# deltaXdeltaQ/QLDPC_Fault_Tolerance

Hardware: AMD Instinct MI355X
Metric: BP-decoded shots/sec (node) on hgp_34_n1600 + % of HBM/LDS roofline (higher is better)
Workload: dtype f64

## Files before the change

### include/qldpc_hip.h

```cpp
#ifndef QLDPC_HIP_H
#define QLDPC_HIP_H

#include <stdint.h>

#ifdef __cplusplus
extern "C" {
#endif

#define QLDPC_ABI_VERSION 1

#define QLDPC_OK 0
#define QLDPC_EINVAL -1
#define QLDPC_EHIP -2
#define QLDPC_ENOMEM -3
#define QLDPC_ENOTSUP -4

#define QLDPC_PRODUCT_SUM 0
#define QLDPC_MIN_SUM 1

#define QLDPC_LOGICAL_X 0
#define QLDPC_LOGICAL_Z 1
#define QLDPC_LOGICAL_TOTAL 2

#define QLDPC_HIST_BINS 1025
// ... 55 lines not shown
int qldpc_osd_gpu_destroy(qldpc_osd_gpu *osd);
int qldpc_osd_gpu_decode(qldpc_osd_gpu *osd, const uint8_t *d_synd, const double *d_post, const uint8_t *d_conv,
                         const uint8_t *d_bp_corr, uint8_t *d_out0, uint8_t *d_outw, int64_t B, void *stream);
typedef struct qldpc_firstmin qldpc_firstmin;
int qldpc_firstmin_create(const qldpc_graph *g, const double *channel_probs, int32_t max_iter,
                          double ms_scaling_factor, int32_t precision, qldpc_firstmin **out);
int qldpc_firstmin_destroy(qldpc_firstmin *fm);
int qldpc_firstmin_decode(qldpc_firstmin *fm, const uint8_t *d_synd, uint8_t *d_corr, int32_t *d_steps, int64_t B,
                          void *stream);

int qldpc_osd_gpu_geometry(const qldpc_osd_gpu *osd, int32_t *row_words, int32_t *window_words, int32_t *threads,
                           int32_t *workgroups);

int qldpc_mc_create(qldpc_bp *dec_x, const qldpc_graph *logical_x, qldpc_bp *dec_z,
                    const qldpc_graph *logical_z, qldpc_mc **out);
int qldpc_mc_destroy(qldpc_mc *mc);

int qldpc_mc_launch(qldpc_mc *mc, double px, double py, double pz, uint64_t seed, uint64_t shot_begin,
                    int64_t shot_count, int32_t logical_mode, const double *d_uniforms, void *d_counters,
                    uint8_t *d_fail, uint8_t *d_err, uint8_t *d_corr, int32_t *d_iters, int32_t grid_blocks,
                    void *stream);

int qldpc_mc_create_staged(qldpc_bp *dec_x, const qldpc_graph *logical_x, qldpc_bp *dec_z,
                           const qldpc_graph *logical_z, qldpc_mc **out);

int qldpc_mc_launch_weight(qldpc_mc *mc, int32_t weight, double px, double py, double pz, uint64_t seed,
                           uint64_t shot_begin, int64_t shot_count, int32_t logical_mode, void *d_counters,
                           uint8_t *d_fail, uint8_t *d_err, uint8_t *d_corr, int32_t *d_iters, void *stream);

int qldpc_mc_run(qldpc_mc *mc, double px, double py, double pz, uint64_t seed, uint64_t shot_begin,
                 int64_t shot_count, int32_t logical_mode, qldpc_counters *out, void *stream);

int qldpc_phenl_create(qldpc_bp *st_x, qldpc_bp *st_z, qldpc_bp *dec2_x, qldpc_bp *dec2_z,
                       const qldpc_graph *logical_x, const qldpc_graph *logical_z, int32_t num_rep, int64_t max_batch,
                       qldpc_phenl **out);
int qldpc_phenl_destroy(qldpc_phenl *ph);
int qldpc_phenl_trace_len(const qldpc_phenl *ph, int32_t num_rounds, int64_t *out);
int qldpc_phenl_launch(qldpc_phenl *ph, double px, double py, double pz, double q, uint64_t seed,
                       uint64_t shot_begin, int64_t shot_count, int32_t num_rounds, int32_t logical_mode,
                       const double *d_uniforms, void *d_counters, uint8_t *d_fail, uint8_t *d_trace, void *stream);

int qldpc_phenl_set_final_osd(qldpc_phenl *ph, qldpc_osd_gpu *osd_x, qldpc_osd_gpu *osd_z);
int qldpc_phenl_set_round_firstmin(qldpc_phenl *ph, qldpc_firstmin *fm_x, qldpc_firstmin *fm_z);

int qldpc_bp_geometry(const qldpc_bp *bp, int32_t *threads, int32_t *vars_per_thread, int32_t *lds_bytes,
                      int32_t *blocks_per_cu);

int qldpc_bp_engine(const qldpc_bp *bp, int32_t *engine);

int qldpc_bp_kernel_id(const qldpc_bp *bp, int32_t *kernel_id, int32_t *row_chunks);

int qldpc_bp_plan(const qldpc_graph *g, const double *channel_probs, int32_t bp_method, int32_t precision,
                  int32_t vars_per_thread, int32_t min_col_slots, int32_t *out, int32_t out_len);

int qldpc_bp_degree3_slots(const qldpc_bp *bp, int32_t *d3k);

int qldpc_bp_create_hbm(qldpc_graph *g, const double *channel_probs, int32_t max_iter, double ms_scaling_factor,
                        int32_t precision, qldpc_bp **out);

int qldpc_bp_create_relay(qldpc_graph *g, const double *channel_probs, int32_t pre_iter, double pre_gamma,
                          int32_t num_legs, int32_t leg_iter, double gamma_lo, double gamma_hi, int32_t stop_nconv,
                          uint64_t gamma_seed, double ms_scaling_factor, int32_t precision, qldpc_bp **out);
int qldpc_relay_gammas(int32_t n, double pre_gamma, int32_t num_legs, double gamma_lo, double gamma_hi,
                       uint64_t gamma_seed, int32_t precision, double *out);
int qldpc_relay_decode_host(int32_t m, int32_t n, const int32_t *row_ptr, const int32_t *col_idx,
                            const double *channel_probs, int32_t pre_iter, double pre_gamma, int32_t num_legs,
                            int32_t leg_iter, double gamma_lo, double gamma_hi, int32_t stop_nconv,
                            uint64_t gamma_seed, double ms_scaling_factor, int32_t precision, const uint8_t *synd,
                            uint8_t *corr, int32_t *iters, uint8_t *conv, int32_t *nsol, int64_t B, int32_t threads);

int qldpc_bp_create_serial(qldpc_graph *g, const double *channel_probs, int32_t max_iter, double ms_scaling_factor,
                           int32_t precision, int32_t soft, qldpc_bp **out);
int qldpc_serial_layers(int32_t m, int32_t n, const int32_t *row_ptr, const int32_t *col_idx, int32_t *layer_out,
                        int32_t *num_layers);
int qldpc_serial_decode_host(int32_t m, int32_t n, const int32_t *row_ptr, const int32_t *col_idx,
                             const double *channel_probs, int32_t max_iter, double ms_scaling_factor,
                             int32_t precision, const uint8_t *synd, uint8_t *corr, int32_t *iters, uint8_t *conv,
                             double *post, int64_t B, int32_t threads);

int qldpc_mc_set_osd(qldpc_mc *mc, qldpc_osd_gpu *osd_x, qldpc_osd_gpu *osd_z);

int qldpc_bp_lds_model(const qldpc_bp *bp, int64_t *out6);
int qldpc_m2s_place_model(const qldpc_graph *g, int32_t anneal_iters, int64_t *out6);
int qldpc_bp_bank_stats(const qldpc_bp *bp, int32_t *before, int32_t *after);

#define QLDPC_COMM_ID_BYTES 128
typedef struct qldpc_comm qldpc_comm;
int qldpc_comm_unique_id(uint8_t *id_out);
int qldpc_comm_init_rank(int device, int32_t nranks, int32_t rank, const uint8_t *id, qldpc_comm **out);
int qldpc_comm_init_all(int32_t ndev, const int32_t *devices, qldpc_comm **out);
int qldpc_comm_rank(const qldpc_comm *comm, int32_t *rank, int32_t *nranks, int32_t *device);
int qldpc_comm_allreduce_counters(qldpc_comm *comm, void *d_counters, void *stream);
int qldpc_comm_allreduce_counters_group(qldpc_comm **comms, void **d_counters, void **streams, int32_t n);
int qldpc_comm_destroy(qldpc_comm *comm);

int qldpc_shard_range(int64_t total, int32_t nparts, int32_t part, int64_t *begin, int64_t *count);
int qldpc_mc_run_sharded(qldpc_mc **mcs, qldpc_comm **comms, int32_t ndev, double px, double py, double pz,
                         uint64_t seed, uint64_t shot_begin, int64_t shot_count, int32_t logical_mode,
                         qldpc_counters *out);

typedef struct qldpc_circ qldpc_circ;
int qldpc_circ_create(const qldpc_graph *dem, const qldpc_graph *dem_obs, const double *probs, qldpc_bp *dec1,
                      const qldpc_graph *h1_space_cor, const qldpc_graph *L1, qldpc_bp *dec2, const qldpc_graph *L2,
                      int32_t num_rounds, int32_t num_rep, int64_t max_batch, qldpc_circ **out);
int qldpc_circ_create_single_shot(const qldpc_graph *dem, const qldpc_graph *dem_obs, const double *probs,
                                  qldpc_bp *dec1, const qldpc_graph *h_space, const qldpc_graph *L1, qldpc_bp *dec2,
                                  const qldpc_graph *L2, int32_t num_cycles, int64_t max_batch, qldpc_circ **out);
int qldpc_circ_set_round_firstmin(qldpc_circ *circ, qldpc_firstmin *fm);
int qldpc_circ_set_final_osd(qldpc_circ *circ, qldpc_osd_gpu *osd_gpu, const qldpc_osd *osd_host);
int qldpc_circ_set_sampler(qldpc_circ *circ, int32_t sampler);
int qldpc_circ_info(const qldpc_circ *circ, int32_t *detectors, int32_t *observables, int32_t *mechanisms);
int qldpc_circ_launch(qldpc_circ *circ, uint64_t seed, uint64_t shot_begin, int64_t shot_count, void *d_counters,
                      uint8_t *d_fail, uint8_t *d_detobs, void *stream);
int qldpc_circ_sample(qldpc_circ *circ, uint64_t seed, uint64_t shot_begin, int64_t shot_count, uint8_t *d_out,
                      void *stream);
int qldpc_circ_destroy(qldpc_circ *circ);

int qldpc_sample_errors(double px, double py, double pz, uint64_t seed, uint64_t shot_begin, int64_t shot_count,
                        int32_t n, const double *d_uniforms, uint8_t *d_err, void *stream);

int qldpc_sample_errors_weight(int32_t weight, double px, double py, double pz, uint64_t seed, uint64_t shot_begin,
                               int64_t shot_count, int32_t n, uint8_t *d_err, void *stream);
int qldpc_sample_errors_weight_host(int32_t weight, double px, double py, double pz, uint64_t seed,
                                    uint64_t shot_begin, int64_t shot_count, int32_t n, uint8_t *err);

typedef struct qldpc_dist qldpc_dist;
int qldpc_dist_create(int device, int32_t rows, int32_t n, int32_t k, const uint64_t *gen_words,
                      const uint64_t *pair_words, qldpc_dist **out);
int qldpc_dist_run_host(qldpc_dist *h, uint64_t seed, uint64_t trial_begin, int64_t trials, int32_t *trial_min,
                        int32_t *best_weight, uint64_t *best_trial, uint64_t *witness_words);
int qldpc_dist_run(qldpc_dist *h, uint64_t seed, uint64_t trial_begin, int64_t trials, int32_t workgroups,
                   int32_t *trial_min, int32_t *best_weight, uint64_t *best_trial, uint64_t *witness_words,
                   void *stream);
int qldpc_dist_geometry(const qldpc_dist *h, int32_t *threads, int32_t *row_words, int32_t *pair_words,
                        int32_t *lds_bytes);
int qldpc_dist_destroy(qldpc_dist *h);

int qldpc_stream_sync(void *stream);

#ifdef __cplusplus
}
#endif
#endif
```

### qldpc_fault_tolerance_amd/_native.py

```python
from __future__ import annotations

import ctypes
import os

PKG_DIR = os.path.dirname(os.path.abspath(__file__))
LIB_PATH = os.environ.get("QLDPC_LIB") or os.path.join(PKG_DIR, "libqldpc_hip.so")
HIST_BINS = 1025

EXPORTED = [
    "qldpc_abi_version", "qldpc_last_error", "qldpc_device_count", "qldpc_graph_create", "qldpc_graph_destroy",
    "qldpc_graph_info", "qldpc_bp_create", "qldpc_bp_destroy", "qldpc_bp_set_channel_probs",
    "qldpc_bp_decode_batch", "qldpc_mc_create", "qldpc_mc_destroy", "qldpc_mc_launch", "qldpc_mc_run",
    "qldpc_bp_geometry", "qldpc_bp_engine", "qldpc_phenl_create", "qldpc_phenl_destroy",
    "qldpc_phenl_trace_len", "qldpc_phenl_launch", "qldpc_bp_degree3_slots", "qldpc_bp_create_soft",
    "qldpc_bp_decode_batch_soft", "qldpc_osd_create", "qldpc_osd_destroy", "qldpc_osd_rank",
    "qldpc_osd_decode_batch", "qldpc_osd_gpu_create", "qldpc_osd_gpu_destroy", "qldpc_osd_gpu_decode", "qldpc_osd_gpu_geometry",
    "qldpc_firstmin_create", "qldpc_firstmin_destroy", "qldpc_firstmin_decode", "qldpc_phenl_set_round_firstmin", "qldpc_phenl_set_final_osd",
    "qldpc_bp_bank_stats", "qldpc_bp_create_hbm", "qldpc_mc_set_osd", "qldpc_comm_unique_id",
    "qldpc_comm_init_rank", "qldpc_comm_init_all", "qldpc_comm_rank", "qldpc_comm_allreduce_counters",
    "qldpc_comm_allreduce_counters_group", "qldpc_comm_destroy", "qldpc_mc_run_sharded", "qldpc_sample_errors",
    "qldpc_stream_sync", "qldpc_bp_kernel_id", "qldpc_build_flags", "qldpc_circ_create", "qldpc_circ_set_final_osd", "qldpc_circ_set_sampler",
    "qldpc_circ_info", "qldpc_circ_launch", "qldpc_circ_sample", "qldpc_circ_destroy",
    "qldpc_shard_range", "qldpc_bp_lds_model", "qldpc_m2s_place_model", "qldpc_bp_plan",
    "qldpc_circ_create_single_shot", "qldpc_circ_set_round_firstmin",
    "qldpc_dist_create", "qldpc_dist_run_host", "qldpc_dist_run", "qldpc_dist_geometry", "qldpc_dist_destroy",
    "qldpc_mc_create_staged", "qldpc_mc_launch_weight", "qldpc_sample_errors_weight",
    "qldpc_sample_errors_weight_host",
    "qldpc_bp_create_relay", "qldpc_relay_gammas", "qldpc_relay_decode_host",
    "qldpc_bp_create_serial", "qldpc_serial_layers", "qldpc_serial_decode_host",
]
BUILD_EXPERIMENTAL = 1
COMM_ID_BYTES = 128


class NativeUnavailable(RuntimeError):
    pass


EINVAL = -1
ENOTSUP = -4


class QldpcError(RuntimeError):

    def __init__(self, msg: str = "", rc: int = 0):
        super().__init__(msg)
        self.rc = rc


class Counters(ctypes.Structure):

    _fields_ = [
        ("shots", ctypes.c_int64),
        ("failures", ctypes.c_int64),
        ("sector_decodes", ctypes.c_int64 * 2),
        ("sector_iters", ctypes.c_int64 * 2),
        ("sector_nonconv", ctypes.c_int64 * 2),
        ("sector_fail", ctypes.c_int64 * 2),
        ("iter_hist", (ctypes.c_int64 * HIST_BINS) * 2),
    ]


COUNTER_WORDS = ctypes.sizeof(Counters) // 8

_lib = None

_vp = ctypes.c_void_p
_i32 = ctypes.c_int32
_i64 = ctypes.c_int64
_u64 = ctypes.c_uint64
_dbl = ctypes.c_double
_pp = ctypes.POINTER(ctypes.c_void_p)


def _declare(L):
    L.qldpc_abi_version.restype = ctypes.c_int
    L.qldpc_abi_version.argtypes = []
    L.qldpc_last_error.restype = ctypes.c_char_p
    L.qldpc_last_error.argtypes = []
    L.qldpc_device_count.restype = ctypes.c_int
    L.qldpc_device_count.argtypes = [ctypes.POINTER(ctypes.c_int)]
    L.qldpc_graph_create.restype = ctypes.c_int
    L.qldpc_graph_create.argtypes = [ctypes.c_int, _i32, _i32, _vp, _vp, _pp]
    L.qldpc_graph_destroy.restype = ctypes.c_int
    L.qldpc_graph_destroy.argtypes = [_vp]
    L.qldpc_graph_info.restype = ctypes.c_int
    L.qldpc_graph_info.argtypes = [_vp] + [ctypes.POINTER(_i32)] * 5
    L.qldpc_bp_create.restype = ctypes.c_int
    L.qldpc_bp_create.argtypes = [_vp, _vp, _i32, _i32, _dbl, _i32, _i32, _i32, _pp]
    L.qldpc_bp_destroy.restype = ctypes.c_int
    L.qldpc_bp_destroy.argtypes = [_vp]
    L.qldpc_bp_set_channel_probs.restype = ctypes.c_int
    L.qldpc_bp_set_channel_probs.argtypes = [_vp, _vp]
    L.qldpc_bp_decode_batch.restype = ctypes.c_int
    L.qldpc_bp_decode_batch.argtypes = [_vp, _vp, _vp, _vp, _vp, _i64, _vp]
    L.qldpc_bp_create_hbm.restype = ctypes.c_int
    L.qldpc_bp_create_hbm.argtypes = [_vp, _vp, _i32, _dbl, _i32, _pp]
    L.qldpc_bp_create_soft.restype = ctypes.c_int
    L.qldpc_bp_create_soft.argtypes = [_vp, _vp, _i32, _dbl, _i32, _pp]
    L.qldpc_bp_decode_batch_soft.restype = ctypes.c_int
    L.qldpc_bp_decode_batch_soft.argtypes = [_vp, _vp, _vp, _vp, _vp, _vp, _i64, _vp]
    L.qldpc_osd_create.restype = ctypes.c_int
    L.qldpc_osd_create.argtypes = [_i32, _i32, _vp, _vp, _vp, _i32, _i32, _pp]
    L.qldpc_osd_destroy.restype = ctypes.c_int
    L.qldpc_osd_destroy.argtypes = [_vp]
    L.qldpc_osd_rank.restype = ctypes.c_int
# ... 13 lines not shown
    L.qldpc_firstmin_decode.restype = ctypes.c_int
    L.qldpc_firstmin_decode.argtypes = [_vp, _vp, _vp, _vp, _i64, _vp]
    L.qldpc_phenl_set_round_firstmin.restype = ctypes.c_int
    L.qldpc_phenl_set_round_firstmin.argtypes = [_vp, _vp, _vp]
    L.qldpc_osd_gpu_geometry.argtypes = [_vp] + [ctypes.POINTER(_i32)] * 4
    L.qldpc_osd_gpu_decode.argtypes = [_vp, _vp, _vp, _vp, _vp, _vp, _vp, _i64, _vp]
    L.qldpc_phenl_set_final_osd.restype = ctypes.c_int
    L.qldpc_phenl_set_final_osd.argtypes = [_vp, _vp, _vp]
    L.qldpc_mc_create.restype = ctypes.c_int
    L.qldpc_mc_create.argtypes = [_vp, _vp, _vp, _vp, _pp]
    L.qldpc_mc_set_osd.restype = ctypes.c_int
    L.qldpc_mc_set_osd.argtypes = [_vp, _vp, _vp]
    L.qldpc_mc_destroy.restype = ctypes.c_int
    L.qldpc_mc_destroy.argtypes = [_vp]
    L.qldpc_mc_launch.restype = ctypes.c_int
    L.qldpc_mc_launch.argtypes = [_vp, _dbl, _dbl, _dbl, _u64, _u64, _i64, _i32, _vp, _vp, _vp, _vp, _vp, _vp,
                                  _i32, _vp]
    L.qldpc_mc_run.restype = ctypes.c_int
    L.qldpc_mc_run.argtypes = [_vp, _dbl, _dbl, _dbl, _u64, _u64, _i64, _i32, ctypes.POINTER(Counters), _vp]
    L.qldpc_bp_geometry.restype = ctypes.c_int
    L.qldpc_bp_geometry.argtypes = [_vp] + [ctypes.POINTER(_i32)] * 4
    L.qldpc_bp_engine.restype = ctypes.c_int
    L.qldpc_bp_engine.argtypes = [_vp, ctypes.POINTER(_i32)]
    L.qldpc_bp_bank_stats.restype = ctypes.c_int
    L.qldpc_bp_bank_stats.argtypes = [_vp, ctypes.POINTER(_i32), ctypes.POINTER(_i32)]
    L.qldpc_bp_degree3_slots.restype = ctypes.c_int
    L.qldpc_bp_degree3_slots.argtypes = [_vp, ctypes.POINTER(_i32)]
    L.qldpc_phenl_create.restype = ctypes.c_int
    L.qldpc_phenl_create.argtypes = [_vp, _vp, _vp, _vp, _vp, _vp, _i32, _i64, _pp]
    L.qldpc_phenl_destroy.restype = ctypes.c_int
    L.qldpc_phenl_destroy.argtypes = [_vp]
    L.qldpc_phenl_trace_len.restype = ctypes.c_int
    L.qldpc_phenl_trace_len.argtypes = [_vp, _i32, ctypes.POINTER(_i64)]
    L.qldpc_phenl_launch.restype = ctypes.c_int
    L.qldpc_phenl_launch.argtypes = [_vp, _dbl, _dbl, _dbl, _dbl, _u64, _u64, _i64, _i32, _i32, _vp, _vp, _vp, _vp,
                                     _vp]
    L.qldpc_comm_unique_id.restype = ctypes.c_int
    L.qldpc_comm_unique_id.argtypes = [_vp]
    L.qldpc_comm_init_rank.restype = ctypes.c_int
    L.qldpc_comm_init_rank.argtypes = [ctypes.c_int, _i32, _i32, _vp, _pp]
    L.qldpc_comm_init_all.restype = ctypes.c_int
    L.qldpc_comm_init_all.argtypes = [_i32, _vp, _pp]
    L.qldpc_comm_rank.restype = ctypes.c_int
    L.qldpc_comm_rank.argtypes = [_vp] + [ctypes.POINTER(_i32)] * 3
    L.qldpc_comm_allreduce_counters.restype = ctypes.c_int
    L.qldpc_comm_allreduce_counters.argtypes = [_vp, _vp, _vp]
    L.qldpc_comm_allreduce_counters_group.restype = ctypes.c_int
    L.qldpc_comm_allreduce_counters_group.argtypes = [_pp, _pp, _pp, _i32]
    L.qldpc_comm_destroy.restype = ctypes.c_int
    L.qldpc_comm_destroy.argtypes = [_vp]
    L.qldpc_mc_run_sharded.restype = ctypes.c_int
    L.qldpc_mc_run_sharded.argtypes = [_pp, _pp, _i32, _dbl, _dbl, _dbl, _u64, _u64, _i64, _i32,
                                       ctypes.POINTER(Counters)]
    L.qldpc_sample_errors.restype = ctypes.c_int
    L.qldpc_sample_errors.argtypes = [_dbl, _dbl, _dbl, _u64, _u64, _i64, _i32, _vp, _vp, _vp]
    L.qldpc_bp_kernel_id.restype = ctypes.c_int
    L.qldpc_bp_kernel_id.argtypes = [_vp, ctypes.POINTER(_i32), ctypes.POINTER(_i32)]
    L.qldpc_bp_plan.restype = ctypes.c_int
    L.qldpc_bp_plan.argtypes = [_vp, _vp, _i32, _i32, _i32, _i32, ctypes.POINTER(_i32), _i32]
    L.qldpc_stream_sync.restype = ctypes.c_int
    L.qldpc_stream_sync.argtypes = [_vp]
    L.qldpc_build_flags.restype = ctypes.c_int
    L.qldpc_build_flags.argtypes = []
    L.qldpc_circ_create.restype = ctypes.c_int
    L.qldpc_circ_create.argtypes = [_vp, _vp, _vp, _vp, _vp, _vp, _vp, _vp, _i32, _i32, _i64, _pp]
    L.qldpc_circ_create_single_shot.restype = ctypes.c_int
    L.qldpc_circ_create_single_shot.argtypes = [_vp, _vp, _vp, _vp, _vp, _vp, _vp, _vp, _i32, _i64, _pp]
    L.qldpc_circ_set_round_firstmin.restype = ctypes.c_int
    L.qldpc_circ_set_round_firstmin.argtypes = [_vp, _vp]
    L.qldpc_circ_set_final_osd.restype = ctypes.c_int
    L.qldpc_circ_set_final_osd.argtypes = [_vp, _vp, _vp]
    L.qldpc_circ_set_sampler.restype = ctypes.c_int
    L.qldpc_circ_set_sampler.argtypes = [_vp, ctypes.c_int32]
    L.qldpc_circ_info.restype = ctypes.c_int
    L.qldpc_circ_info.argtypes = [_vp] + [ctypes.POINTER(_i32)] * 3
    L.qldpc_circ_launch.restype = ctypes.c_int
    L.qldpc_circ_launch.argtypes = [_vp, _u64, _u64, _i64, _vp, _vp, _vp, _vp]
    L.qldpc_circ_sample.restype = ctypes.c_int
    L.qldpc_circ_sample.argtypes = [_vp, _u64, _u64, _i64, _vp, _vp]
    L.qldpc_bp_lds_model.restype = ctypes.c_int
    L.qldpc_bp_lds_model.argtypes = [_vp, ctypes.POINTER(_i64)]
    L.qldpc_m2s_place_model.restype = ctypes.c_int
    L.qldpc_m2s_place_model.argtypes = [_vp, ctypes.c_int32, ctypes.POINTER(_i64)]
    L.qldpc_shard_range.restype = ctypes.c_int
    L.qldpc_shard_range.argtypes = [_i64, _i32, _i32, ctypes.POINTER(_i64), ctypes.POINTER(_i64)]
    L.qldpc_circ_destroy.restype = ctypes.c_int
    L.qldpc_circ_destroy.argtypes = [_vp]
    L.qldpc_dist_create.restype = ctypes.c_int
    L.qldpc_dist_create.argtypes = [ctypes.c_int, _i32, _i32, _i32, _vp, _vp, _pp]
    L.qldpc_dist_run_host.restype = ctypes.c_int
    L.qldpc_dist_run_host.argtypes = [_vp, _u64, _u64, _i64, _vp, ctypes.POINTER(_i32), ctypes.POINTER(_u64), _vp]
    L.qldpc_dist_run.restype = ctypes.c_int
    L.qldpc_dist_run.argtypes = [_vp, _u64, _u64, _i64, _i32, _vp, ctypes.POINTER(_i32), ctypes.POINTER(_u64), _vp,
                                 _vp]
    L.qldpc_dist_geometry.restype = ctypes.c_int
    L.qldpc_dist_geometry.argtypes = [_vp] + [ctypes.POINTER(_i32)] * 4
    L.qldpc_dist_destroy.restype = ctypes.c_int
    L.qldpc_dist_destroy.argtypes = [_vp]
    L.qldpc_mc_create_staged.restype = ctypes.c_int
    L.qldpc_mc_create_staged.argtypes = [_vp, _vp, _vp, _vp, _pp]
    L.qldpc_mc_launch_weight.restype = ctypes.c_int
    L.qldpc_mc_launch_weight.argtypes = [_vp, _i32, _dbl, _dbl, _dbl, _u64, _u64, _i64, _i32, _vp, _vp, _vp, _vp,
                                         _vp, _vp]
    L.qldpc_sample_errors_weight.restype = ctypes.c_int
    L.qldpc_sample_errors_weight.argtypes = [_i32, _dbl, _dbl, _dbl, _u64, _u64, _i64, _i32, _vp, _vp]
    L.qldpc_sample_errors_weight_host.restype = ctypes.c_int
    L.qldpc_sample_errors_weight_host.argtypes = [_i32, _dbl, _dbl, _dbl, _u64, _u64, _i64, _i32, _vp]
    relay = [_i32, _dbl, _i32, _i32, _dbl, _dbl, _i32, _u64, _dbl, _i32]
    L.qldpc_bp_create_relay.restype = ctypes.c_int
    L.qldpc_bp_create_relay.argtypes = [_vp, _vp] + relay + [_pp]
    L.qldpc_relay_gammas.restype = ctypes.c_int
    L.qldpc_relay_gammas.argtypes = [_i32, _dbl, _i32, _dbl, _dbl, _u64, _i32, _vp]
    L.qldpc_relay_decode_host.restype = ctypes.c_int
    L.qldpc_relay_decode_host.argtypes = [_i32, _i32, _vp, _vp, _vp] + relay + [_vp, _vp, _vp, _vp, _vp, _i64, _i32]
    L.qldpc_bp_create_serial.restype = ctypes.c_int
    L.qldpc_bp_create_serial.argtypes = [_vp, _vp, _i32, _dbl, _i32, _i32, _pp]
    L.qldpc_serial_layers.restype = ctypes.c_int
    L.qldpc_serial_layers.argtypes = [_i32, _i32, _vp, _vp, _vp, _vp]
    L.qldpc_serial_decode_host.restype = ctypes.c_int
    L.qldpc_serial_decode_host.argtypes = [_i32, _i32, _vp, _vp, _vp, _i32, _dbl, _i32, _vp, _vp, _vp, _vp, _vp, _i64,
                                           _i32]


def lib():
    global _lib
    if _lib is None:
        if not os.path.exists(LIB_PATH):
            raise NativeUnavailable(
                f"{LIB_PATH} not found: build the HIP extension first (__graft_entry__.build()); "
                "the engine has no CPU fallback")
        import torch

        L = ctypes.CDLL(LIB_PATH)
        _declare(L)
        if L.qldpc_abi_version() != 1:
            raise NativeUnavailable("libqldpc_hip.so ABI version mismatch")
        _lib = L
    return _lib


def check(rc: int, what: str = "") -> None:
    if rc != 0:
        msg = lib().qldpc_last_error().decode(errors="replace")
        raise QldpcError(f"{what} failed (rc={rc}): {msg}", rc)


def experimental_families() -> bool:
    return bool(lib().qldpc_build_flags() & BUILD_EXPERIMENTAL)


def device_count() -> int:
    c = ctypes.c_int(0)
    rc = lib().qldpc_device_count(ctypes.byref(c))
    return c.value if rc == 0 else 0


def require_gpu() -> None:
    if device_count() <= 0:
        raise NativeUnavailable("no HIP device visible: the MI355X engine needs a GPU (no CPU fallback)")
```

### qldpc_fault_tolerance_amd/csrc/bp_reg.h

```cpp
#pragma once

#ifndef QLDPC_TID_LAUNDER
#define QLDPC_TID_LAUNDER 1
#endif
#ifndef QLDPC_STAMPS
#define QLDPC_STAMPS 0
#endif
#ifndef QLDPC_FLIP_BRANCHFREE
#define QLDPC_FLIP_BRANCHFREE 0
#endif
#ifndef QLDPC_FLIPLATE
#define QLDPC_FLIPLATE 0
#endif
#ifndef QLDPC_M2S_MBCNT
#define QLDPC_M2S_MBCNT 0
#endif
#ifndef QLDPC_C2S_PF
#define QLDPC_C2S_PF 2
#endif
#ifndef QLDPC_F32_C2V4
#define QLDPC_F32_C2V4 1
#endif
#ifndef QLDPC_F64_C2V5
#define QLDPC_F64_C2V5 1
#endif
#ifndef QLDPC_ABS_SH2
#define QLDPC_ABS_SH2 1
#endif
#ifndef QLDPC_C2S_W128
#define QLDPC_C2S_W128 1
#endif
#ifndef QLDPC_M2S_UNIL
#define QLDPC_M2S_UNIL 1
#endif
#ifndef QLDPC_M2S_KEEPVA
#define QLDPC_M2S_KEEPVA 1
#endif
#ifndef QLDPC_M2S_RPTR
#define QLDPC_M2S_RPTR 1
#endif
#ifndef QLDPC_RC_RPTR
#define QLDPC_RC_RPTR 1
#endif
#ifndef QLDPC_M2S_ROWPAIR
#define QLDPC_M2S_ROWPAIR 0
#endif
#ifndef QLDPC_M2S_XMASK
#define QLDPC_M2S_XMASK 1
#endif
#include "bp_slot.h"

namespace qldpc {

constexpr int eng_base(int E) { return E % 10; }
constexpr int eng_sh(int E) { return (E / 10) % 10 ? 2 : 0; }
constexpr bool eng_kv64(int E) { return (E / 100) % 10 != 0; }
constexpr int eng_tail(int E) { return (E / 1000) % 10; }
constexpr bool eng_m2s(int E) { return (E / 10000) % 10 == 1 || (E / 10000) % 10 == 4; }
constexpr bool eng_m2v(int E) { return (E / 10000) % 10 == 4; }
template <int D3K>
__host__ __device__ constexpr int m2v_ecnt(int k) { return 3 * (k < D3K ? k : D3K) + 4 * (k > D3K ? k - D3K : 0); }
constexpr int kM2vRows = 4;
constexpr bool eng_fb(int E) { return (E / 10000) % 10 == 2; }
constexpr bool eng_c2s(int E) { return (E / 10000) % 10 == 3; }
constexpr int eng_d2k(int E) { return (E / 100000) % 10; }
constexpr bool eng_nw(int E) { return eng_m2s(E) && !eng_m2v(E) && eng_tail(E) && eng_sh(E) == 2; }
constexpr int kNwSlots = 2;
template <int ENG, int D3K>
__device__ constexpr bool no_edge(int k, int t) {
  return (eng_m2s(ENG) || eng_c2s(ENG) || eng_fb(ENG)) && ((k < D3K && t >= 3) || (k < eng_d2k(ENG) && t >= 2));
}
constexpr bool eng_m2x(int E) { return eng_m2s(E) || eng_c2s(E); }
template <typename T, int ENG>
constexpr int lb_waves(int LB) {
  return LB <= 256 ? (sizeof(T) == 8 ? (eng_m2s(ENG) && (ENG / 100) % 10 == 2 ? 4
                                        : (eng_base(ENG) == 4 || eng_m2x(ENG)) ? 3 : 2) : 4)
                   : (LB <= 512 && (eng_kv64(ENG) || eng_fb(ENG))) ? 4 : 1;
}
__device__ inline unsigned long long qstamp() {
#if QLDPC_STAMPS
  unsigned long long t;
  __builtin_amdgcn_sched_barrier(0);
  asm volatile("s_memtime %0\n\ts_waitcnt lgkmcnt(0)" : "=s"(t) : : "memory");
  __builtin_amdgcn_sched_barrier(0);
  return t;
#else
  return 0;
#endif
}
template <int ENG>
__device__ inline uint32_t ea_cs(uint32_t ea) { return (ea & 0xFFFFu) << eng_sh(ENG); }
template <int ENG>
__device__ inline uint32_t ea_v(uint32_t ea) { return (ea >> 16) << eng_sh(ENG); }

struct RLayout {
  uint32_t v, t, f, sink, lred, total;
};

__host__ __device__ inline RLayout r_layout(int eng, int vslots, int mmax, int tsize, int tail = 0, int m2s = 0,
                                            int fb = 0) {
  RLayout L;
  L.v = eng == 4 ? 0u : (uint32_t)a16((size_t)(mmax + 1) * (m2s == 2 ? 0 : m2s ? 1 : 2) * tsize);
  L.t = L.v + (uint32_t)a16((size_t)vslots * tsize);
  L.f = L.t + (tail ? (uint32_t)a16((size_t)mmax * tsize) : 0u);
  L.sink = L.f + (uint32_t)a16((size_t)(mmax + 1) * (fb ? 1 : 4));
  L.lred = L.sink + (eng == 4 ? 16u : 0u);
  L.total = L.lred + 48;
  return L;
}
__host__ __device__ inline size_t r_lds_bytes(int img, int chunk) {
  return (size_t)img + 2 * a16((size_t)((chunk + 31) / 32) * 4) + 8 * 12;
}

template <typename T>
struct CSEntry {
  using type = Pair<T>;
};

template <typename T>
__device__ inline T& lds_at(unsigned char* smem, uint32_t off) {
  return *reinterpret_cast<T*>(smem + off);
}
template <typename X>
using LdsPtr = __attribute__((address_space(3))) X*;
__device__ inline uint32_t lds_base(unsigned char* smem) {
  return (uint32_t)(uintptr_t)(LdsPtr<unsigned char>)smem;
}
template <int B>
struct LdsWord;
template <>
struct LdsWord<4> {
  typedef uint32_t type;
};
template <>
struct LdsWord<8> {
  typedef uint32_t type __attribute__((ext_vector_type(2)));
};
template <>
struct LdsWord<16> {
  typedef uint32_t type __attribute__((ext_vector_type(4)));
};
// ... 822 lines not shown
      if (TAIL) r.tcur = lds_ld<T, AP>(smem, r.toff);
      r.fcur = lds_ld<uint32_t, AP>(smem, r.fo);
    }
  };
  auto reduce_row = [&](const RowIn& r, int qq) {
    uint32_t s;
    if (FIRST) {
      s = ((r.fcur >> 1) ^ (r.fcur >> 2)) & 1u;
      sbits |= s << qq;
      lds_st<uint32_t, AP>(smem, r.fo, (r.fcur & 4u) | ((r.fcur >> 2) & 1u));
    } else {
      s = (sbits >> qq) & 1u;
      mism |= (int)((r.fcur ^ s) & 1u);
    }
    double f1 = FT<T>::val(FT<T>::kSent), f2 = f1;
    uint32_t px = s ? 0x80000000u : 0u;
    uint32_t aoff = coff[0];
#pragma unroll
    for (int c = 0; c < NCH; ++c) {
#pragma unroll
      for (int k = 0; k < NV; ++k) {
        const double x = V16<T>::get(r.cur[c], k);
        aoff = __builtin_fabs(x) < f1 ? coff[c] + 8u * (uint32_t)k : aoff;
        double t;
        asm("v_max_f64 %0, %1, |%2|" : "=v"(t) : "v"(f1), "v"(x));
        asm("v_min_f64 %0, %1, %2" : "=v"(f2) : "v"(f2), "v"(t));
        asm("v_min_f64 %0, %1, |%2|" : "=v"(f1) : "v"(f1), "v"(x));
      }
      uint32_t p;
      asm("v_bitop3_b32 %0, %1, %2, %3 bitop3:0x96"
          : "=v"(p)
          : "v"(px), "v"((uint32_t)(FT<T>::bits(r.cur[c].x) >> 32)), "v"((uint32_t)(FT<T>::bits(r.cur[c].y) >> 32)));
      px = p;
    }
    uint32_t amin = r.roff + aoff;
    if (TAIL) {
      const double x = (double)r.tcur;
      amin = __builtin_fabs(x) < f1 ? r.toff : amin;
      double t;
      asm("v_max_f64 %0, %1, |%2|" : "=v"(t) : "v"(f1), "v"(x));
      asm("v_min_f64 %0, %1, %2" : "=v"(f2) : "v"(f2), "v"(t));
      asm("v_min_f64 %0, %1, |%2|" : "=v"(f1) : "v"(f1), "v"(x));
      px ^= (uint32_t)(FT<T>::bits(r.tcur) >> 32);
    }
    const U par = (U)(px & 0x80000000u) << 32;
    lds_st<U, AP>(smem, r.co, FT<T>::bits(f1) | par);
    lds_st<U, AP>(smem, amin, FT<T>::bits(f2) | par);
  };
  const uint32_t drb = (uint32_t)TB * rstride, dtp = (uint32_t)TB * (uint32_t)sizeof(T), dfp = 4u * (uint32_t)TB,
                 dcp = (uint32_t)TB * (uint32_t)sizeof(T);
  if constexpr (QLDPC_M2S_ROWPAIR > 0 && TAIL && NCH == 4) {
    for (int i = tid; i < m; i += 2 * TB, q += 2) {
      if constexpr (AP) asm volatile("" : "+v"(rb));
      RowIn a, b;
      load_row(a, i, rb, tp, fp, cp);
      const bool hb = i + TB < m;
      constexpr int PC = QLDPC_M2S_ROWPAIR < NCH ? QLDPC_M2S_ROWPAIR : NCH;
      if (hb) load_row(b, i + TB, rb + drb, tp + dtp, fp + dfp, cp + dcp, 0, PC);
      reduce_row(a, q);
      if (hb) {
        if constexpr (PC < NCH) load_row(b, i + TB, rb + drb, tp + dtp, fp + dfp, cp + dcp, PC, NCH);
        reduce_row(b, q + 1);
      }
      rb += 2 * drb;
      tp += 2 * dtp;
      fp += 2 * dfp;
      cp += 2 * dcp;
    }
  } else {
    for (int i = tid; i < m; i += TB, ++q) {
      if constexpr (AP) asm volatile("" : "+v"(rb));
      RowIn a;
      load_row(a, i, rb, tp, fp, cp);
      reduce_row(a, q);
      rb += drb;
      tp += dtp;
      fp += dfp;
      cp += dcp;
    }
  }
  return mism;
}

template <typename T, bool FIRST>
__device__ inline int m2v_check(unsigned char* smem, const RLayout& Ly, int m, int tid, int TB, uint32_t& sbits,
                                const M2vRows& RW, uint32_t vbase) {
  using U = typename FT<T>::U;
  static_assert(sizeof(T) == 8, "m2v: fp64 only");
  int mism = 0;
#pragma unroll
  for (int q = 0; q < kM2vRows; ++q) {
    const int i = tid + q * TB;
    if (i >= m) break;
    const uint32_t wd[4] = {RW.w[q].x, RW.w[q].y, RW.w[q].z, RW.w[q].w};
    uint32_t a[7];
#pragma unroll
    for (int e = 0; e < 7; ++e) a[e] = vbase + ((e & 1) ? (wd[e >> 1] >> 16) : (wd[e >> 1] & 0xFFFFu));
    double x[7];
#pragma unroll
    for (int e = 0; e < 7; ++e) x[e] = FT<T>::val(lds_ld<U, true>(nullptr, a[e]));
    const uint32_t fo = Ly.f + 4u * (uint32_t)(i + 1);
    const uint32_t fcur = lds_at<uint32_t>(smem, fo);
    uint32_t s;
    if (FIRST) {
      s = ((fcur >> 1) ^ (fcur >> 2)) & 1u;
      sbits |= s << q;
      lds_at<uint32_t>(smem, fo) = (fcur & 4u) | ((fcur >> 2) & 1u);
    } else {
      s = (sbits >> q) & 1u;
      mism |= (int)((fcur ^ s) & 1u);
    }
    double f1 = FT<T>::val(FT<T>::kSent), f2 = f1;
    uint32_t px = s ? 0x80000000u : 0u;
    uint32_t amin = a[0];
#pragma unroll
    for (int e = 0; e < 7; ++e) {
      amin = __builtin_fabs(x[e]) < f1 ? a[e] : amin;
      double t;
      asm("v_max_f64 %0, %1, |%2|" : "=v"(t) : "v"(f1), "v"(x[e]));
      asm("v_min_f64 %0, %1, %2" : "=v"(f2) : "v"(f2), "v"(t));
      asm("v_min_f64 %0, %1, |%2|" : "=v"(f1) : "v"(f1), "v"(x[e]));
    }
#pragma unroll
    for (int e = 0; e + 1 < 7; e += 2) {
      uint32_t p;
      asm("v_bitop3_b32 %0, %1, %2, %3 bitop3:0x96"
          : "=v"(p)
          : "v"(px), "v"((uint32_t)(FT<T>::bits(x[e]) >> 32)), "v"((uint32_t)(FT<T>::bits(x[e + 1]) >> 32)));
      px = p;
    }
    px ^= (uint32_t)(FT<T>::bits(x[6]) >> 32);
    const U par = (U)(px & 0x80000000u) << 32;
    lds_at<U>(smem, (uint32_t)(i + 1) * (uint32_t)sizeof(T)) = FT<T>::bits(f1) | par;
    lds_st<U, true>(nullptr, amin, FT<T>::bits(f2) | par);
  }
  return mism;
}

template <typename T, bool FIRST, int NCH, int TAIL>
__device__ inline int c2s_check(unsigned char* smem, const RLayout& Ly, int m, int wtid, int TB, uint32_t& sbits,
                                T alpha) {
  using U = typename FT<T>::U;
  using VT = typename V16<T>::type;
  constexpr int NV = V16<T>::N;
  static_assert(sizeof(T) == 8, "c2s: fp64 only");
  int mism = 0;
  int q = 0;
  int tid = wtid;
  asm volatile("" : "+v"(tid));
  const uint32_t rstride = (uint32_t)NCH * 16u;
  for (int i = tid; i < m; i += TB, ++q) {
    const uint32_t roff = Ly.v + 16u + (uint32_t)i * rstride;
    VT cur[NCH];
#pragma unroll
    for (int c = 0; c < NCH; ++c) cur[c] = *reinterpret_cast<const VT*>(smem + roff + 16u * (uint32_t)c);
    const uint32_t toff = Ly.t + (uint32_t)i * (uint32_t)sizeof(T);
    T tcur = (T)0;
    if (TAIL) tcur = lds_at<T>(smem, toff);
    const uint32_t fcur = lds_at<uint32_t>(smem, Ly.f + 4u * (uint32_t)(i + 1));
    uint32_t s;
    if (FIRST) {
      s = ((fcur >> 1) ^ (fcur >> 2)) & 1u;
      sbits |= s << q;
      lds_at<uint32_t>(smem, Ly.f + 4u * (uint32_t)(i + 1)) = (fcur & 4u) | ((fcur >> 2) & 1u);
    } else {
      s = (sbits >> q) & 1u;
// ... 204 lines not shown
    lds_at<Pair<T>>(smem, 0) = z;
  }
}

template <typename T>
constexpr int kRowChunks4 = 8 * (int)sizeof(T) / 16;
template <typename T, bool FIRST>
__device__ inline int c_check_any(unsigned char* smem, const RLayout& Ly, int m, int nch, int tid, int TB,
                                  uint32_t& sbits, T alpha) {
  (void)nch;
  return c_check<T, FIRST, kRowChunks4<T>>(smem, Ly, m, tid, TB, sbits, alpha);
}

template <typename T, int DMAX, int VPL, bool MC, int ENG, int D3K, int NCH = 0>
__device__ void r_pass(const SSector& S, int q, long long c0, int cn, unsigned char* smem, const RLayout& Ly,
                       int vslots, int mmax, uint32_t* failmap, unsigned long long* cnt, const SMcArgs* A,
                       const SDecArgs* D, int tid, int TB) {
  using U = typename FT<T>::U;
  constexpr bool KV = RState<T, DMAX, VPL, ENG>::kKeepV;
  const int m = S.m, n = S.n, nch = S.nch;
  int tidp = tid;
#if QLDPC_TID_LAUNDER
  asm volatile("" : "+v"(tidp));
#endif
  RState<T, DMAX, VPL, ENG> R;
  constexpr bool SP = RState<T, DMAX, VPL, ENG>::kSplit;
  const int wbase = (int)__builtin_amdgcn_readfirstlane((uint32_t)tid) & ~63;
  const uint32_t sbase = lds_base(smem);
  r_load<T, DMAX, VPL, ENG>(S, R, Ly, tidp, TB, sbase);
  r_fill<T, ENG>(S, smem, Ly, vslots, mmax, tidp, TB);
  FMap M;
  M.fbase = eng_base(ENG) == 4 ? Ly.f + 4u : Ly.f;
  M.rstart = Ly.v + 16u;
  M.rsh = 4 + __builtin_ctz((unsigned)nch);
  constexpr bool AB = RState<T, DMAX, VPL, ENG>::kAbs;
  if (AB) M.fbase = Ly.f - (sbase >> (eng_fb(ENG) ? 3 : (sizeof(T) == 4 || eng_m2s(ENG)) ? 1 : 2));
  const uint32_t fdelta = eng_base(ENG) == 4 ? Ly.f : M.fbase;
  const bool last_live = eng_nw(ENG) ? ((S.live_last >> ((uint32_t)wbase >> 6)) & 1u) != 0
                                     : uni((VPL - 1) * TB + (tid & ~63) < S.npos ? 1 : 0) != 0;
  uint32_t nwm = 0;
  if constexpr (eng_nw(ENG)) {
    const uint32_t wv = (uint32_t)wbase >> 6;
#pragma unroll
    for (int k = 0; k < kNwSlots && k < VPL; ++k) nwm |= ((S.nw >> (16 * k + wv)) & 1u) << k;
    nwm = __builtin_amdgcn_readfirstlane(nwm);
  }
  uint32_t* lred = reinterpret_cast<uint32_t*>(smem + Ly.lred);
  uint32_t* flags = lred + 8;
  const bool adaptive = S.alpha == 0.0;
  const T alpha_fixed = (T)S.alpha;
  __syncthreads();

  int pshot = -1, pit = 0, pconv = 0;
  unsigned long long st_acc[10] = {0, 0, 0, 0, 0, 0, 0, 0, 0, 0};
  unsigned long long st_a = qstamp();
  for (int sh = 0; sh <= cn; ++sh) {
    const bool have = sh < cn;
    uint32_t eb = 0, sb = 0;
    r_launder<T, DMAX, VPL, ENG, D3K>(R);
    int tidl = tid;
    asm volatile("" : "+v"(tidl));
    if (have) {
#pragma unroll
      for (int k = 0; k < VPL; ++k) {
        const U cl = FT<T>::bits(r_prior(R, k));
#pragma unroll
        for (int t = 0; t < DMAX; ++t) {
          if (no_edge<ENG, D3K>(k, t)) continue;
          if constexpr (eng_m2v(ENG)) {
            if (k == VPL - 1 && tidl >= S.vnl) continue;
            lds_st<U, true>(smem, m2v_va<T, DMAX, VPL, ENG, D3K, 256>(R, k, t), cl);
          }
          else
            lds_st<U, AB>(smem, r_va(R, k, t), cl);
          if (KV) R.ov[KV ? k : 0][KV ? t : 0] = cl;
        }
      }
      if (MC) {
        const long long sl = c0 + sh;
        const unsigned long long gshot = A->shot_begin + (unsigned long long)sl;
        int jv[VPL];
#pragma unroll
        for (int k = 0; k < VPL; ++k) jv[k] = S.perm[k * TB + tidl];
        uint16_t* cc = nullptr;
        bool cc_read = false;
        uint32_t cw = 0;
        if (A->cls_cache && !A->uniforms && VPL <= 8) {
          cc = A->cls_cache + ((long long)blockIdx.x * A->chunk + sh) * TB + tidl;
          cc_read = q == A->sec_id1;
          if (cc_read) cw = *cc;
        }
#pragma unroll
        for (int k = 0; k < VPL; ++k) {
          const int j = jv[k];
          if (j >= 0) {
            uint32_t cls;
            if (A->uniforms) {
              const double u = A->uniforms[sl * (long long)n + j];
              cls = (u < A->t1) ? 2u : (A->t1 <= u && u < A->t2) ? 1u : (A->t2 <= u && u < A->t3) ? 3u : 0u;
            } else if (cc_read) {
              cls = (cw >> (2 * k)) & 3u;
            } else {
              const unsigned long long kk = philox_k53(A->seed, gshot, (uint32_t)j);
              cls = (kk < A->K1) ? 2u : (kk < A->K2) ? 1u : (kk < A->K3) ? 3u : 0u;
              cw |= cls << (2 * k);
            }
            const uint32_t e = (q == 0) ? (cls & 1u) : (cls >> 1);
            eb |= e << k;
            if (A->err && q == A->sec_id0) A->err[sl * (long long)n + j] = (uint8_t)cls;
            if (e) {
#pragma unroll
              for (int t = 0; t < DMAX; ++t) {
                if (no_edge<ENG, D3K>(k, t)) continue;
                if constexpr (eng_base(ENG) == 4)
                  atomicXor(&lds_at<uint32_t>(smem, f_addr<T, ENG>(R.ea[k][t], M)), 2u);
                else if constexpr (eng_c2s(ENG))
                  lds_xor_abs(R.ea[k][t], 2u);
                else
                  f_xor<ENG>(smem, r_fa(R, k, t, M.fbase), 2u);
              }
            }
          }
        }
        if (cc && !cc_read) *cc = (uint16_t)cw;
      } else {
        const uint8_t* srow = D->synd + (c0 + sh) * (long long)m;
        for (int i = tidl; i < m; i += TB) {
          const uint32_t fo = f_off<ENG>(Ly, i + 1);
          const uint32_t F = f_ld<ENG>(smem, fo);
          const int oi = S.rperm ? S.rperm[i] : i;
          f_st<ENG>(smem, fo, (eng_base(ENG) == 4 ? (F & 0xFFFF0000u) : (F & 4u)) | ((uint32_t)(srow[oi] & 1u) << 1));
        }
      }
    }
    if (QLDPC_STAMPS) {
      const unsigned long long t = qstamp();
      st_acc[4] += t - st_a;
      st_a = t;
    }
    M2vRows rwv;
    if constexpr (eng_m2v(ENG))
      if (have) m2v_rows_load(S, tid, TB, m, rwv);
    __syncthreads();
    if (pshot >= 0) {
      uint32_t lf = 0;
      if (MC) {
#pragma unroll
        for (int w = 0; w < 8; ++w) lf |= lred[w];
      }
      const int f = (!pconv || lf) ? 1 : 0;
      if (tid == 0) {
        const long long sl = c0 + pshot;
        if (MC) {
          if (f) failmap[pshot >> 5] |= 1u << (pshot & 31);
          cnt[kCntDec + q] += 1;
          cnt[kCntIters + q] += (unsigned long long)pit;
          cnt[kCntNonconv + q] += pconv ? 0 : 1;
          cnt[kCntSecFail + q] += (unsigned long long)f;
          atomicAdd(&A->counters[kCntHist + q * kHistBins + (pit < kHistBins ? pit : kHistBins - 1)], 1ull);
          if (A->iters) A->iters[sl * 2 + q] = pit;
        } else {
          if (D->iters) D->iters[sl] = pit;
          if (D->conv) D->conv[sl] = pconv ? 1 : 0;
        }
      }
    }
    if (!have) break;
    if (QLDPC_STAMPS) {
      const unsigned long long t = qstamp();
      st_acc[8] += t - st_a;
      st_a = t;
    }
    if constexpr (eng_base(ENG) == 4)
      c_check_any<T, true>(smem, Ly, m, nch, tid, TB, sb, adaptive ? (T)0.5 : alpha_fixed);
    else if constexpr (eng_c2s(ENG))
      c2s_check<T, true, NCH, eng_tail(ENG)>(smem, Ly, m, tid, TB, sb, adaptive ? (T)0.5 : alpha_fixed);
    else if constexpr (eng_m2v(ENG))
      m2v_check<T, true>(smem, Ly, m, tid, TB, sb, rwv, sbase + Ly.v);
    else if constexpr (eng_m2s(ENG))
      m_check<T, true, NCH, eng_tail(ENG)>(smem, Ly, m, wbase, tid, TB, sb);
    else if constexpr (NCH > 0)
      r_check_c<T, true, NCH, eng_tail(ENG), QLDPC_PFC, ENG>(smem, Ly, m, tid, TB, sb);
    else
      r_check<T, true>(smem, Ly, m, nch, tid, TB, sb, adaptive ? (T)0.5 : alpha_fixed);
    __syncthreads();
    if (tid < 10) lred[tid] = 0;
    if (QLDPC_STAMPS) {
      const unsigned long long t = qstamp();
      st_acc[9] += t - st_a;
      st_acc[7] += 1;
      st_a = t;
    }
    int it = 1;
    bool conv = false;
    uint32_t xb = 0;
    uint64_t xm[VPL];
#pragma unroll
    for (int k = 0; k < VPL; ++k) xm[k] = 0;
    long long cslot = -1;
    while (true) {
      int mism;
      double* cpost = nullptr;
      if constexpr (MC && eng_base(ENG) == 3) {
        if (A->c_n && A->c_post[q] && it >= S.max_iter) {
          uint32_t* s_cslot = lred + 11;
          if (tid == 0) *s_cslot = atomicAdd(&A->c_n[q], 1u);
          __syncthreads();
          cslot = (long long)*s_cslot;
          if (cslot < A->c_cap) cpost = A->c_post[q] + cslot * (long long)n;
        }
      }
      if constexpr (eng_base(ENG) == 4) {
        xb = c_var<T, DMAX, VPL>(smem, R, M, last_live);
        __syncthreads();
        const T alpha = adaptive ? (T)(1.0 - ldexp(1.0, -(it + 1))) : alpha_fixed;
        mism = c_check_any<T, false>(smem, Ly, m, nch, tid, TB, sb, alpha);
      } else {
        const T alpha = adaptive ? (T)(1.0 - ldexp(1.0, -it)) : alpha_fixed;
        constexpr int kPV = (eng_tail(ENG) && !eng_m2x(ENG) && !eng_fb(ENG)) ? 0 : QLDPC_PRIO_V;
        if (kPV) __builtin_amdgcn_s_setprio(kPV);
        if constexpr (eng_m2x(ENG))
          xb = m_var<T, DMAX, VPL, D3K, ENG>(smem, R, fdelta, alpha, xb, xm, last_live, cpost, S.perm + tidl, TB, nwm);
        else
          xb = r_var<T, DMAX, VPL, D3K, ENG>(smem, R, fdelta, alpha, xb, last_live, cpost, S.perm + tidl, TB);
        if (kPV) __builtin_amdgcn_s_setprio(0);
        if constexpr (eng_m2v(ENG)) m2v_rows_load(S, tid, TB, m, rwv);
        unsigned long long t1 = 0;
        if (QLDPC_STAMPS) {
          t1 = qstamp();
          st_acc[0] += t1 - st_a;
        }
        __syncthreads();
        if (QLDPC_STAMPS) {
          st_a = qstamp();
          st_acc[1] += st_a - t1;
        }
        const T alpha_next = adaptive ? (T)(1.0 - ldexp(1.0, -(it + 1))) : alpha_fixed;
        if (QLDPC_PRIO_C) __builtin_amdgcn_s_setprio(QLDPC_PRIO_C);
        if constexpr (eng_c2s(ENG))
          mism = c2s_check<T, false, NCH, eng_tail(ENG)>(smem, Ly, m, tid, TB, sb, alpha_next);
        else if constexpr (eng_m2v(ENG))
          mism = m2v_check<T, false>(smem, Ly, m, tid, TB, sb, rwv, sbase + Ly.v);
        else if constexpr (eng_m2s(ENG))
          mism = m_check<T, false, NCH, eng_tail(ENG)>(smem, Ly, m, wbase, tid, TB, sb);
        else if constexpr (NCH > 0)
          mism = r_check_c<T, false, NCH, eng_tail(ENG), QLDPC_PFC, ENG>(smem, Ly, m, tid, TB, sb);
        else
          mism = r_check<T, false>(smem, Ly, m, nch, tid, TB, sb, alpha_next);
        if (QLDPC_PRIO_C) __builtin_amdgcn_s_setprio(0);
        if (QLDPC_STAMPS) {
          const unsigned long long t = qstamp();
          st_acc[2] += t - st_a;
          st_a = t;
        }
      }
      if (__any(mism) && (tid & 63) == 0) flags[it & 1] = 1u;
      __syncthreads();
      if (QLDPC_STAMPS) {
        const unsigned long long t = qstamp();
        st_acc[3] += t - st_a;
        st_acc[6] += 1;
        st_a = t;
      }
      const int any = uni((int)flags[it & 1]);
      if (tid == 0) flags[(it & 1) ^ 1] = 0;
      conv = any == 0;
      if (conv || it >= S.max_iter) break;
      ++it;
    }
    if constexpr (eng_m2x(ENG) && eng_base(ENG) != 4 && m_xmask(ENG)) {
      xb = 0;
#pragma unroll
      for (int k = 0; k < VPL; ++k) xb |= (__builtin_amdgcn_inverse_ballot_w64(xm[k]) ? 1u : 0u) << k;
    }
    const long long sl = c0 + sh;
    if (MC && cslot >= 0 && cslot < A->c_cap) {
      if (!conv) {
        uint8_t* cs = A->c_synd[q] + cslot * (long long)m;
        int qq = 0;
        for (int i = tidl; i < m; i += TB, ++qq)
          cs[S.rperm ? S.rperm[i] : i] =
              (uint8_t)(((sb >> qq) ^ (f_ld<ENG>(smem, f_off<ENG>(Ly, i + 1)) >> 2)) & 1u);
        uint8_t* ce = A->c_err[q] + cslot * (long long)n;
#pragma unroll
        for (int k = 0; k < VPL; ++k) {
          const int j = S.perm[k * TB + tidl];
          if (j >= 0) ce[j] = (uint8_t)((eb >> k) & 1u);
        }
      }
      if (tid == 0) A->c_shot[q][cslot] = conv ? -1 : sl;
    }
    if (MC) {
      const uint32_t r = eb ^ xb;
      if (__any(r != 0)) {
        int jv[VPL];
#pragma unroll
        for (int k = 0; k < VPL; ++k) jv[k] = ((r >> k) & 1u) ? S.perm[k * TB + tidl] : -1;
        const int kw = S.kw;
#pragma unroll
        for (int w = 0; w < 4; ++w) {
          if (w >= kw) break;
          unsigned long long lm[VPL];
#pragma unroll
          for (int k = 0; k < VPL; ++k) lm[k] = jv[k] >= 0 ? S.lmask[(long long)jv[k] * kw + w] : 0ull;
          unsigned long long a = 0;
#pragma unroll
          for (int k = 0; k < VPL; ++k) a ^= lm[k];
          const uint32_t lo = wave_xor_u32((uint32_t)a), hi = wave_xor_u32((uint32_t)(a >> 32));
          if ((tid & 63) == 0) {
            if (lo) atomicXor(&lred[2 * w], lo);
            if (hi) atomicXor(&lred[2 * w + 1], hi);
          }
        }
      }
      if (A->corr) {
#pragma unroll
        for (int k = 0; k < VPL; ++k) {
          const int j = S.perm[k * TB + tidl];
          if (j >= 0) A->corr[(sl * 2 + q) * (long long)n + j] = (uint8_t)((xb >> k) & 1u);
        }
      }
    } else {
#pragma unroll
      for (int k = 0; k < VPL; ++k) {
        const int j = S.perm[k * TB + tidl];
// ... 106 lines not shown
```

### qldpc_fault_tolerance_amd/csrc/bp_slot.h

```cpp
#pragma once
#include "bp_kernels.h"

namespace qldpc {

constexpr int kMaxThreadsS = 1024;
constexpr int kMaxVplS = 32;
constexpr uint32_t kNoEdgeS = 0u;
__device__ inline uint32_t echk(uint32_t e) { return e & 0xFFFFu; }
__device__ inline uint32_t eslot(uint32_t e) { return e >> 16; }

struct SSector {
  const uint32_t* edges;
  const void* llr;
  const unsigned long long* lmask;
  const uint8_t* rdeg;
  const int32_t* perm;
  const int32_t* rperm;
  int m, n, kw, max_iter, nch, vpl;
  int d3k;
  double alpha;
  const uint32_t* rows;
  int vlast, vnl;
  int npos;
  uint32_t nw;
  uint32_t live_last;
};

struct SMcArgs {
  SSector sec[2];
  int nsec, sec_id0, sec_id1, logical_mode;
  int mmax, vslots, img_bytes, chunk;
  unsigned long long K1, K2, K3;
  double t1, t2, t3;
  unsigned long long seed, shot_begin;
  long long shot_count;
  const double* uniforms;
  unsigned long long* counters;
  uint8_t* fail;
  uint8_t* err;
  uint8_t* corr;
  int* iters;
  unsigned int* work;
  unsigned int* c_n;
  double* c_post[2];
  uint8_t* c_synd[2];
  uint8_t* c_err[2];
  long long* c_shot[2];
  long long c_cap;
  unsigned long long* stamps;
  uint16_t* cls_cache;
};

struct SDecArgs {
  SSector sec;
  const uint8_t* synd;
  uint8_t* corr;
  int* iters;
  uint8_t* conv;
  long long B;
  int mmax, vslots, img_bytes, chunk;
  unsigned int* work;
  unsigned long long* stamps;
};

template <typename T> struct V16;
template <> struct V16<float> {
  using type = float4;
  static constexpr int N = 4;
  __device__ static inline float get(const float4& v, int k) { return k == 0 ? v.x : k == 1 ? v.y : k == 2 ? v.z : v.w; }
  __device__ static inline float4 splat(float s) { return make_float4(s, s, s, s); }
};
template <> struct V16<double> {
  using type = double2;
  static constexpr int N = 2;
  __device__ static inline double get(const double2& v, int k) { return k == 0 ? v.x : v.y; }
  __device__ static inline double2 splat(double s) { return make_double2(s, s); }
};

__host__ __device__ inline size_t a16(size_t x) { return (x + 15) & ~(size_t)15; }

__host__ __device__ inline size_t slot_img_bytes(int vslots, int mmax, int tsize) {
  return a16((size_t)vslots * tsize) + a16((size_t)(mmax + 1) * 2 * tsize) + a16((size_t)(mmax + 1) * 4) + 48;
}
__host__ __device__ inline size_t slot_lds_bytes(int ns, int img, int chunk) {
  return (size_t)ns * img + 2 * a16((size_t)((chunk + 31) / 32) * 4) + 8 * 12;
}

template <typename T>
struct Img {
  T* V;
  Pair<T>* CS;
  uint32_t* F;
  uint32_t* lred;
  uint32_t* flags;
};

template <typename T>
__device__ inline Img<T> slot_img(unsigned char* smem, int q, int img_bytes, int vslots, int mmax) {
  unsigned char* b = smem + (size_t)q * img_bytes;
  Img<T> I;
  I.V = reinterpret_cast<T*>(b);
  size_t off = a16((size_t)vslots * sizeof(T));
  I.CS = reinterpret_cast<Pair<T>*>(b + off);
  off += a16((size_t)(mmax + 1) * 2 * sizeof(T));
  I.F = reinterpret_cast<uint32_t*>(b + off);
  off += a16((size_t)(mmax + 1) * 4);
  I.lred = reinterpret_cast<uint32_t*>(b + off);
  I.flags = I.lred + 8;
  return I;
}

template <typename T>
__device__ inline typename FT<T>::U canon(T v) {
  using U = typename FT<T>::U;
  return (FT<T>::bits(v) & ~FT<T>::kSign) | ((v <= (T)0) ? FT<T>::kSign : (U)0);
}

template <int DMAX>
__device__ inline void load_edges(const SSector& S, int k, int tid, int TB, uint32_t (&e)[DMAX]) {
#pragma unroll
  for (int t = 0; t < DMAX; ++t) e[t] = S.edges[(k * DMAX + t) * TB + tid];
}

template <typename T, int DMAX>
__device__ inline void s_priors(const SSector& S, T* V, int tid, int TB) {
  const T* llr = static_cast<const T*>(S.llr);
  for (int k = 0; k < S.vpl; ++k) {
    uint32_t e[DMAX];
    load_edges<DMAX>(S, k, tid, TB, e);
    const T c = FT<T>::val(canon<T>(llr[k * TB + tid]));
#pragma unroll
    for (int t = 0; t < DMAX; ++t) V[eslot(e[t])] = c;
  }
// ... 372 lines not shown
```

### qldpc_fault_tolerance_amd/csrc/qldpc_hip.hip

```cpp
#include <hip/hip_runtime.h>

#include <algorithm>
#include <cmath>
#include <cstdio>
#include <cstdlib>
#include <cstring>
#include <map>
#include <mutex>
#include <string>
#include <vector>

#include "../../include/qldpc_hip.h"
#include "variants.h"
#include "runtime.h"

using namespace qldpc;
using namespace qldpc_rt;

thread_local std::string qldpc_rt::g_err;

namespace {

const int kVplSet[] = {1, 2, 3, 4, 5, 6, 7, 8, 10, 12};
constexpr int kLdsMax = 160 * 1024;
constexpr int kChunkMax = 1024;

int env_int(const char* name, int dflt) {
  const char* e = std::getenv(name);
  return (e && *e) ? std::atoi(e) : dflt;
}

}

namespace {

Variant get_variant(int precision, int vpl, int dmax) {
  if (precision == 32) return dmax == 4 ? get_variant_f32_d4(vpl) : get_variant_f32_d8(vpl);
  return dmax == 4 ? get_variant_f64_d4(vpl) : get_variant_f64_d8(vpl);
}

SVariant get_svariant(int precision, int dmax, int ns) {
  if (precision == 32) return dmax == 4 ? get_svariant_f32_d4(ns) : get_svariant_f32_d8(ns);
  return dmax == 4 ? get_svariant_f64_d4(ns) : get_svariant_f64_d8(ns);
}

SVariant get_rvariant(int engine, int precision, int vpl, int d3k, int dmax) {
  if (engine == 4) return precision == 32 ? get_r4variant_f32(vpl) : get_r4variant_f64(vpl);
  if (precision == 32 && dmax == 5) return get_rvariant_f32_d5(vpl, d3k);
  if (precision == 32 && dmax == 6) return get_rvariant_f32_d6(vpl, d3k);
  return precision == 32 ? get_rvariant_f32(vpl, d3k) : get_rvariant_f64(vpl);
}

bool use_f64w(const Route& r) {
  return r.engine == 3 && r.precision == 64 &&
         (r.DMAX == 4 || (r.DMAX == 5 && (r.VPL <= 5 || (r.VPL == 6 && r.nch == 5)))) && r.ea_shift == 0 && r.TB <= 256 &&
         r.VPL >= 4 && r.VPL <= 8 && (r.nch == 3 || r.nch == 4 || (r.DMAX == 5 && r.nch == 5)) &&
         env_int("QLDPC_F64W", 1) != 0;
}

bool use_f32w(const Route& r) {
  return r.engine == 3 && r.precision == 32 && r.DMAX == 4 && r.ea_shift == 0 && r.VPL >= 5 && r.VPL <= 8 && r.nch == 2 &&
         env_int("QLDPC_F32W", 1) != 0;
}

#if QLDPC_STAMPS
unsigned long long* debug_stamps_buffer() {
  static unsigned long long* buf = nullptr;
  if (!buf && hipMalloc(&buf, 10 * sizeof(unsigned long long)) == hipSuccess) (void)hipMemset(buf, 0, 80);
  return buf;
}
#endif

bool use_f64x(const Route& r) {
  return r.engine == 3 && r.precision == 64 && r.DMAX == 4 && r.ea_shift == 0 && r.TB > 256 && r.TB <= 512 && r.VPL >= 3 &&
         r.VPL <= 4 && QLDPC_EXPERIMENTAL && env_int("QLDPC_F64X", 0) != 0;
}

SVariant slot_variant(const Route& r) {
  const SVariant none{nullptr, nullptr, nullptr, nullptr};
  const bool e3 = r.engine == 3, f64 = r.precision == 64;
  if (r.fb) {
    const bool ok = e3 && !f64 && r.DMAX == 4 && r.ea_shift == 2 && r.nch == 2 && r.tail && r.TB == 512;
    return ok ? get_rvariant_f32_stfb(r.VPL, r.d3k, r.d2k) : none;
  }
  if (r.m2s) {
    if (r.m2s == 1 && e3 && f64 && r.DMAX == 4 && r.ea_shift == 2 && r.nch == 4 && r.tail && r.TB >= 512)
      return get_rvariant_f64_m2st(r.VPL, r.d3k, r.d2k);
    if (r.m2s == 1 && e3 && f64 && r.DMAX == 5 && r.ea_shift == 0 && r.nch == 4 && !r.tail && r.TB <= 256)
      return r.m2s_pk ? get_rvariant_f64_m2s8pk(r.VPL, r.d3k) : get_rvariant_f64_m2s8(r.VPL, r.d3k);
    const bool ok = e3 && f64 && r.DMAX == 4 && r.ea_shift == 0 && r.nch == 3 && r.tail && r.TB <= 256;
    if (r.m2s == 3)
      return (e3 && f64 && r.DMAX == 4 && r.ea_shift == 0 && r.TB == 256) ? get_rvariant_f64_m2v(r.VPL, r.d3k) : none;
    if (!ok) return none;
    return r.m2s == 2 ? get_rvariant_f64_c2s(r.VPL, r.d3k) : get_rvariant_f64_m2s(r.VPL, r.d3k);
  }
  if (r.tail) {
    const bool ok = e3 && r.DMAX == 4 && r.ea_shift == 2 && r.nch == (f64 ? 4 : 2) && (r.TB > 512 || (f64 && r.TB == 512));
    if (!ok) return none;
    return f64 ? get_rvariant_f64_st(r.VPL, r.d3k, r.d2k) : get_rvariant_f32_st(r.VPL, r.d3k);
  }
  if (use_f64w(r)) return r.DMAX == 5 ? get_rvariant_f64_w_d5(r.VPL, r.d3k, r.nch) : get_rvariant_f64_w(r.VPL, r.d3k, r.nch);
  if (use_f64x(r)) return get_rvariant_f64_x(r.VPL, r.d3k);
  if (use_f32w(r)) return get_rvariant_f32_w(r.VPL, r.d3k);
  if (r.engine == 4 && f64 && r.TB <= 256 && r.VPL >= 4) return get_r4variant_f64_w(r.VPL);
  if (e3 && r.ea_shift == 2) return (!f64 && r.DMAX == 4) ? get_rvariant_f32_big(r.VPL, r.d3k) : none;
  return r.engine >= 3 ? get_rvariant(r.engine, r.precision, r.VPL, r.d3k, r.DMAX) : get_svariant(r.precision, r.DMAX, r.NS);
}

int route_kernel_id(const Route& r) {
  if (r.engine != 3) return r.engine;
  if (r.m2s)
    return r.m2s == 2 ? 31103 : r.m2s == 3 ? 40103 : (r.tail && r.nch == 4) ? 11313 + 100000 * std::min(r.d2k, 1)
           : r.tail ? 11103 : r.m2s_pk ? 10203 : 10103;
  if (r.fb) return 21013 + ((r.d3k >= 8 && r.d2k > 0) ? 100000 * std::min(r.d2k, 4) : 0);
  if (r.tail) return 1013 + ((r.precision == 64 && r.VPL == 6 && r.d2k >= 1 && r.d3k >= 1) ? 100000 : 0);
  return use_f64w(r) ? 103 : use_f64x(r) ? 303 : r.ea_shift == 2 ? 13 : 3;
}

int round_up(int x, int a) { return (x + a - 1) / a * a; }

int max_spill_free_vpl(int precision, int dmax) {
  if (precision == 32) return dmax == 4 ? 10 : 5;
  return dmax == 4 ? 6 : 3;
}

int choose_geometry(int n, int m, int requested_vpl, int vmax, int& TB, int& VPL) {
  if (requested_vpl > 0) {
    bool ok = false;
    for (int v : kVplSet) ok |= (v == requested_vpl);
    if (!ok) return set_err(QLDPC_EINVAL, "vars_per_thread must be one of 1-8,10,12");
    VPL = requested_vpl;
    TB = round_up((n + VPL - 1) / VPL, 64);
    if (TB > kMaxThreads) return set_err(QLDPC_EINVAL, "vars_per_thread too small for this graph (>512 threads)");
  } else {
    double best = 1e30;
    for (int v : kVplSet) {
      const int tb = round_up((n + v - 1) / v, 64);
      if (tb > kMaxThreads || v > vmax) continue;
      const double waste = (double)(tb * v - n) / (double)(tb * v);
      const double score = waste + (v < 4 ? 0.25 : 0.0) + 0.01 * v;
      if (score < best) {
        best = score;
        TB = tb;
        VPL = v;
      }
    }
    if (best >= 1e30) return set_err(QLDPC_ENOTSUP, "graph too large for the register-resident kernel");
  }
  if ((m + TB - 1) / TB > 32) return set_err(QLDPC_ENOTSUP, "too many checks per thread (m > 32*threads)");
  return 0;
}

size_t lds_for(int precision, int mmax) {
  const size_t pair = precision == 32 ? 8 : 16;
  return pair * 2 * (size_t)mmax + 4 * 2 * (size_t)mmax + 64;
}

int choose_sgeometry(int n, int m, int requested_vpl, int& TB, int& VPL) {
  const int forced_tb = env_int("QLDPC_TB", 0);
  if (requested_vpl > 0) {
    VPL = requested_vpl;
    TB = round_up((n + VPL - 1) / VPL, 64);
  } else if (forced_tb > 0) {
    TB = round_up(forced_tb, 64);
    VPL = (n + TB - 1) / TB;
  } else {
    TB = std::min(256, round_up(n, 64));
    VPL = (n + TB - 1) / TB;
    if (VPL > kMaxVplS) {
      TB = std::min(kMaxThreadsS, round_up((n + kMaxVplS - 1) / kMaxVplS, 64));
      VPL = (n + TB - 1) / TB;
    }
  }
  if (TB > kMaxThreadsS || TB < 64) return set_err(QLDPC_EINVAL, "threads per shot out of range (64..1024)");
  if (VPL > kMaxVplS) return set_err(QLDPC_ENOTSUP, "more than 32 variables per thread (n > 32768)");
  if ((m + TB - 1) / TB > 32) return set_err(QLDPC_ENOTSUP, "too many checks per thread (m > 32*threads)");
  return 0;
}

constexpr int kMaxVplR = 8;
constexpr int kPrefVplR = 7;
int choose_rgeometry(int n, int m, int requested_vpl, int& TB, int& VPL, int pref = kPrefVplR, int vmax = kMaxVplR) {
  const int forced_tb = env_int("QLDPC_TB", 0);
  if (requested_vpl > 0) {
    VPL = requested_vpl;
    TB = round_up((n + VPL - 1) / VPL, 64);
  } else if (forced_tb > 0) {
    TB = round_up(forced_tb, 64);
    VPL = (n + TB - 1) / TB;
  } else {
    TB = 64;
    while (TB < kMaxThreadsS && ((n + TB - 1) / TB > pref || (m + TB - 1) / TB > 32)) TB *= 2;
    VPL = (n + TB - 1) / TB;
  }
  if (TB > kMaxThreadsS || TB < 64 || VPL < 1 || VPL > vmax || (m + TB - 1) / TB > 32) return 1;
  return 0;
}

RLayout route_layout(const Route& r, int vslots, int mmax) {
  return r_layout(r.engine, vslots, mmax, r.precision == 32 ? 4 : 8, r.tail, r.m2s, r.fb);
}
size_t route_lds(const Route& r, int vslots, int mmax) {
  return r_lds_bytes((int)route_layout(r, vslots, mmax).total, kChunkMax);
}

bool route_fits(const Route& r, int vslots, int mmax) {
  return route_layout(r, vslots, mmax).lred <= (65536u << r.ea_shift) && route_lds(r, vslots, mmax) <= (size_t)kLdsMax;
}

int choose_ns(int img) {
  const int forced = env_int("QLDPC_NS", 1);
  const int ns = (forced == 2 || forced == 4) ? forced : 1;
  return slot_lds_bytes(ns, img, kChunkMax) <= (size_t)kLdsMax ? ns : 1;
}

int device_cus(int dev, int& cus) {
  hipDeviceProp_t prop;
  QLDPC_HIP(hipGetDeviceProperties(&prop, dev));
  cus = prop.multiProcessorCount;
  return 0;
}

}

extern "C" {

#if QLDPC_STAMPS
int qldpc_debug_stamps(unsigned long long* out) {
  unsigned long long* b = debug_stamps_buffer();
  if (!b || hipDeviceSynchronize() != hipSuccess || hipMemcpy(out, b, 80, hipMemcpyDeviceToHost) != hipSuccess) return -1;
  return hipMemset(b, 0, 80) == hipSuccess ? 0 : -1;
}
#endif

int qldpc_abi_version(void) { return QLDPC_ABI_VERSION; }

const char* qldpc_last_error(void) { return qldpc_rt::g_err.c_str(); }

int qldpc_build_flags(void) { return QLDPC_EXPERIMENTAL ? QLDPC_BUILD_EXPERIMENTAL : 0; }

int qldpc_device_count(int* out) {
  if (!out) return set_err(QLDPC_EINVAL, "out is NULL");
  int c = 0;
  hipError_t e = hipGetDeviceCount(&c);
  if (e != hipSuccess) {
    *out = 0;
    return set_err(QLDPC_EHIP, std::string("hipGetDeviceCount: ") + hipGetErrorString(e));
  }
  *out = c;
  return 0;
}

int qldpc_graph_create(int device, int32_t m, int32_t n, const int32_t* row_ptr, const int32_t* col_idx,
                       qldpc_graph** out) {
  if (!out || !row_ptr || (m > 0 && !col_idx)) return set_err(QLDPC_EINVAL, "NULL argument");
  if (m < 0 || n <= 0) return set_err(QLDPC_EINVAL, "bad shape");
  if (m >= 0xFFFF) return set_err(QLDPC_ENOTSUP, "more than 65534 checks");
  if (row_ptr[0] != 0) return set_err(QLDPC_EINVAL, "row_ptr[0] != 0");
  auto* g = new qldpc_graph();
  g->device = device;
  g->m = m;
  g->n = n;
  g->nnz = row_ptr[m];
  g->row_ptr.assign(row_ptr, row_ptr + m + 1);
  g->col_idx.assign(col_idx, col_idx + g->nnz);
  g->col_rows.assign(n, {});
  for (int i = 0; i < m; ++i) {
    if (row_ptr[i + 1] < row_ptr[i]) {
      delete g;
      return set_err(QLDPC_EINVAL, "row_ptr not monotone");
    }
    g->max_row = std::max(g->max_row, row_ptr[i + 1] - row_ptr[i]);
    for (int e = row_ptr[i]; e < row_ptr[i + 1]; ++e) {
      const int c = col_idx[e];
      if (c < 0 || c >= n || (e > row_ptr[i] && col_idx[e - 1] >= c)) {
        delete g;
        return set_err(QLDPC_EINVAL, "col_idx out of range or not strictly ascending within a row");
      }
      g->col_rows[c].push_back(i);
    }
  }
  for (int j = 0; j < n; ++j) g->max_col = std::max<int>(g->max_col, (int)g->col_rows[j].size());
  *out = g;
// ... 600 lines not shown
    delete bp;
    return code;
  };
  const int E = g->nnz;
  int rc;
  if ((rc = upload_csr_csc(bp)) || (rc = bp->llr.alloc((size_t)g->n * (precision == 32 ? 4 : 8)))) return fail(rc);
  if ((rc = upload_llr(bp))) return fail(rc);
  const bool lds_msgs = ps_lds_bytes(precision, g->m, g->n, E, true) <= 96 * 1024;
  bp->route.lds_bytes = (int)ps_lds_bytes(precision, g->m, g->n, E, lds_msgs);
  if (bp->route.lds_bytes > kLdsMax) return fail(set_err(QLDPC_ENOTSUP, "graph too large for the product-sum engine"));
  int nb = 0;
  if (hipOccupancyMaxActiveBlocksPerMultiprocessor(&nb, ps_kernel(precision), bp->route.TB, bp->route.lds_bytes) != hipSuccess)
    nb = 1;
  bp->blocks_per_cu = std::max(1, nb);
  if ((rc = device_cus(g->device, bp->cus))) return fail(rc);
  bp->ps_grid = (long long)bp->blocks_per_cu * bp->cus;
  if (!lds_msgs && (rc = bp->ps_ws.alloc((size_t)bp->ps_grid * 2 * E * (precision == 32 ? 4 : 8)))) return fail(rc);
  *out = bp;
  return 0;
}

static int create_min_sum(qldpc_graph* g, const double* channel_probs, int32_t max_iter, int32_t bp_method,
                          double ms_scaling_factor, int32_t precision, int32_t vars_per_thread,
                          int32_t min_col_slots, int forced_engine, qldpc_bp** out);

static void bp1_prepare(qldpc_bp* bp) {
  if (bp->bp1) {
    qldpc_firstmin_destroy(bp->bp1);
    bp->bp1 = nullptr;
  }
  bp->bp1_off = !(bp->max_iter == 1 && bp->method == 1) || bp->route.engine >= 7 || env_int("QLDPC_BP1", 1) == 0;
  if (bp->bp1_off) return;
  const std::string keep = qldpc_rt::g_err;
  if (qldpc_firstmin_create(bp->g, bp->probs.data(), 0, bp->alpha, bp->route.precision, &bp->bp1) != 0) {
    bp->bp1 = nullptr;
    bp->bp1_off = true;
    qldpc_rt::g_err = keep;
  }
}

int qldpc_bp_create(qldpc_graph* g, const double* channel_probs, int32_t max_iter, int32_t bp_method,
                    double ms_scaling_factor, int32_t precision, int32_t vars_per_thread, int32_t min_col_slots,
                    qldpc_bp** out) {
  return create_min_sum(g, channel_probs, max_iter, bp_method, ms_scaling_factor, precision, vars_per_thread,
                        min_col_slots, 0, out);
}

int qldpc_bp_create_hbm(qldpc_graph* g, const double* channel_probs, int32_t max_iter, double ms_scaling_factor,
                        int32_t precision, qldpc_bp** out) {
  return create_min_sum(g, channel_probs, max_iter, QLDPC_MIN_SUM, ms_scaling_factor, precision, 0, 0, 6, out);
}

int qldpc_bp_create_soft(qldpc_graph* g, const double* channel_probs, int32_t max_iter, double ms_scaling_factor,
                         int32_t precision, qldpc_bp** out) {
  return create_min_sum(g, channel_probs, max_iter, QLDPC_MIN_SUM, ms_scaling_factor, precision, 0, 0, 1, out);
}


static bool uniform_priors(const double* probs, int n) {
  for (int j = 1; j < n; ++j)
    if (probs[j] != probs[0]) return false;
  return true;
}

static int validate_create(const qldpc_graph* g, const double* channel_probs, int precision, int bp_method) {
  if (!g || !channel_probs) return set_err(QLDPC_EINVAL, "NULL argument");
  if (precision != 32 && precision != 64) return set_err(QLDPC_EINVAL, "precision must be 32 or 64");
  if (bp_method != QLDPC_MIN_SUM && bp_method != QLDPC_PRODUCT_SUM)
    return set_err(QLDPC_EINVAL, "bp_method must be 0 (product_sum) or 1 (minimum_sum)");
  if (g->m <= 0) return set_err(QLDPC_EINVAL, "a decoder needs at least one check (m = 0)");
  return 0;
}

static bool fits(const Route& c, const qldpc_graph* g) { return route_fits(c, route_vslots(c, g->m), g->m); }

static int to_hbm(const qldpc_graph* g, Route& r, std::vector<int32_t>& slot_var, const char* why = nullptr) {
  if (why && env_int("QLDPC_HBM_FALLBACK", 1) == 0) return set_err(QLDPC_ENOTSUP, why);
  if (g->max_row > kHbmMaxDeg || g->max_col > kHbmMaxDeg)
    return set_err(QLDPC_ENOTSUP, "HBM engine: row or column degree above 12");
  r.engine = 6;
  r.TB = kHbmThreads;
  r.VPL = 1;
  r.lds_bytes = 0;
  r.ea_shift = r.tail = r.m2s = r.fb = r.m2s_pk = r.vslots_dummy = r.d3k = r.d2k = 0;
  r.nw = r.live_last = 0;
  slot_var.clear();
  return 0;
}

static void admit_tail(const qldpc_graph* g, int vars_per_thread, Route& r) {
  const bool f64t = r.precision == 64 && env_int("QLDPC_E3_TAIL64", 1) != 0;
  Route plain = r;
  plain.ea_shift = f64t ? 0 : 2;
  if (!(r.engine == 3 && r.DMAX == 4 && (g->max_row == 9 || (f64t && g->max_row == 8)) && env_int("QLDPC_E3_TAIL", 1) != 0 &&
        (r.precision == 32 || !fits(plain, g))))
    return;
  Route c = r;
  c.tail = 1;
  c.nch = r.precision == 32 ? 2 : 4;
  c.ea_shift = 2;
  Route fb = c;
  fb.fb = 1;
  fb.TB = 512;
  fb.VPL = (g->n + 511) / 512;
  int tb = 0, vpl = 0;
  if (r.precision == 32 && vars_per_thread <= 0 && env_int("QLDPC_TB", 0) <= 0 && env_int("QLDPC_E3_FB", 1) != 0 &&
      fb.VPL >= 9 && fb.VPL <= 12 && (g->m + 511) / 512 <= 32 && fits(fb, g) &&
      2 * route_lds(fb, route_vslots(fb, g->m), g->m) <= (size_t)kLdsMax)
    r = fb;
  else if (fits(c, g) && !choose_rgeometry(g->n, g->m, vars_per_thread, tb, vpl) && (tb > 512 || (f64t && tb == 512)) &&
           vpl >= 4 && vpl <= 8)
    r = c;
}

static void admit_m2s(const qldpc_graph* g, bool uniform, int vars_per_thread, Route& r) {
  if (!(r.engine == 3 && r.precision == 64 && r.DMAX == 4 && !r.tail && g->max_row >= 1 && g->max_row <= 7 &&
        env_int("QLDPC_M2S", 1) != 0 && env_int("QLDPC_DEGSORT", 1) != 0))
    return;
  int tb = 0, vpl = 0, n3 = 0, nother = 0;
  for (int j = 0; j < g->n; ++j) {
    const int d = (int)g->col_rows[j].size();
    n3 += d == 3;
    nother += d != 3 && d != 4;
  }
  Route c = r;
  c.tail = 1;
  c.m2s = 1;
  c.nch = 3;
  c.ea_shift = 0;
  if (nother || !uniform || choose_rgeometry(g->n, g->m, vars_per_thread, tb, vpl) || tb > 256 || vpl < 4 || vpl > 8 ||
      !(n3 % tb == 0 || n3 == g->n) || !fits(c, g))
    return;
  r = c;
  bool full = true;
  for (int i = 0; i < g->m && full; ++i) full = g->row_ptr[i + 1] - g->row_ptr[i] == 7;
  c.m2s = 2;
  if (full && QLDPC_EXPERIMENTAL && env_int("QLDPC_C2S", 0) != 0 && fits(c, g)) r.m2s = 2;
  const int d3 = n3 == g->n ? vpl : n3 / 256;
  const int nlast = g->n - (vpl - 1) * 256, NL = (nlast + 63) & ~63;
  const int ecl = 3 * std::min(vpl - 1, d3) + 4 * std::max(0, vpl - 1 - d3);
  Route v = r;
  v.m2s = 3;
  v.tail = 0;
  v.vslots_m2v = ecl * 256 + (vpl - 1 < d3 ? 3 : 4) * NL + 1;
  v.m2v_vlast = ecl * 256;
  v.m2v_nl = NL;
  if (r.m2s == 1 && tb == 256 && g->m <= 4 * 256 && v.vslots_m2v * 8 < 65536 && QLDPC_EXPERIMENTAL &&
      env_int("QLDPC_M2V", 0) != 0 && fits(v, g))
    r = v;
}

static void admit_m2st(const qldpc_graph* g, bool uniform, int vars_per_thread, Route& r) {
  if (!(r.engine == 3 && r.precision == 64 && r.DMAX == 4 && r.tail && !r.fb && !r.m2s && r.nch == 4 &&
        env_int("QLDPC_M2ST", 1) != 0 && env_int("QLDPC_DEGSORT", 1) != 0 && env_int("QLDPC_D2K", 1) != 0))
    return;
  int tb = 0, vpl = 0;
  if (!uniform || choose_rgeometry(g->n, g->m, vars_per_thread, tb, vpl) || tb < 512) return;
  const StPlan P = st_plan(g, tb, vpl, r.DMAX, env_int("QLDPC_NW", 1) != 0, env_int("QLDPC_NW_BAL", 1) != 0);
  Route c = r;
  c.m2s = 1;
  c.vslots_dummy = P.nd;
  c.nw = P.nw;
  c.live_last = P.live_last;
#if QLDPC_DIAG_NOLAST
  c.live_last = 0;
#endif
  if (g->max_col <= r.DMAX && P.d2 >= 1 && route_vslots(c, g->m) < 0x3FFFF && get_rvariant_f64_m2st(vpl, P.d3, P.d2).dec_k &&
      fits(c, g))
    r = c;
}

static void admit_d5_256(const qldpc_graph* g, const Route& r, int pref, int& vars_per_thread, int& vmax) {
  if (!(r.engine == 3 && r.precision == 64 && r.DMAX == 5 && vars_per_thread <= 0 && env_int("QLDPC_TB", 0) <= 0 &&
        env_int("QLDPC_D5_256", 1) != 0 && g->max_row > 8 && g->max_row <= 10))
    return;
  int tb = 0, vpl = 0;
  if (choose_rgeometry(g->n, g->m, 0, tb, vpl, pref, vmax) || tb <= 256) return;
  for (int v = 5; v <= 6 && vars_per_thread <= 0; ++v) {
    int tb5 = 0, vpl5 = 0;
    if (!choose_rgeometry(g->n, g->m, v, tb5, vpl5, pref, 6) && tb5 <= 256) {
      vars_per_thread = v;
      vmax = std::max(vmax, v);
    }
  }
}

static void admit_m2s8(const qldpc_graph* g, bool uniform, int pref, int vmax, int& vars_per_thread, Route& r) {
  if (!(r.engine == 3 && r.precision == 64 && r.DMAX == 5 && !r.tail && !r.m2s && g->max_row >= 1 && g->max_row <= 8 &&
        env_int("QLDPC_M2S", 1) != 0 && env_int("QLDPC_M2S8", 1) != 0 && env_int("QLDPC_DEGSORT", 1) != 0))
    return;
  int tb = 0, vpl = 0, n3 = 0, small_vpt = 0;
  for (int j = 0; j < g->n; ++j) n3 += g->col_rows[j].size() <= 3;
  if (!uniform || choose_rgeometry(g->n, g->m, vars_per_thread, tb, vpl, pref, vmax)) return;
  if (tb == 256 && vpl < 4 && vars_per_thread <= 0 && env_int("QLDPC_TB", 0) <= 0 && env_int("QLDPC_M2S8_SMALL", 1) != 0)
    for (int v = std::min(6, vmax); v >= 4 && !small_vpt; --v) {
      int tb2 = 0, vpl2 = 0;
      if (!choose_rgeometry(g->n, g->m, v, tb2, vpl2, pref, vmax) && tb2 < 256 && vpl2 == v) {
        tb = tb2;
        vpl = vpl2;
        small_vpt = v;
      }
    }
  if (!((tb == 256 || (tb < 256 && small_vpt > 0)) && vpl >= 4 && vpl <= 6)) return;
  const int d3 = n3 == g->n ? vpl : n3 / tb;
  const std::vector<int32_t> order = degree_sorted(g, {3});
  Route c = r;
  c.m2s = 1;
  c.nch = 4;
  c.ea_shift = 0;
  for (int p = 0; p < g->n; ++p) c.vslots_dummy += ((p / tb) < d3 ? 3 : r.DMAX) - (int)g->col_rows[order[p]].size();
  if (route_vslots(c, g->m) >= 0xFFFF || !fits(c, g)) return;
  r = c;
  if (small_vpt > 0) vars_per_thread = small_vpt;
  r.m2s_pk = env_int("QLDPC_M2S8_PK", 1) != 0 && vpl <= 5 && 4 * route_lds(c, route_vslots(c, g->m), g->m) <= (size_t)kLdsMax;
}

static int plan_route(const qldpc_graph* g, bool uniform, int precision, int vars_per_thread, int min_col_slots,
                      int forced_engine, Route& r, std::vector<int32_t>& slot_var) {
  const int want_engine = forced_engine ? forced_engine : env_int("QLDPC_ENGINE", 3);
  if (want_engine == 4 && !QLDPC_EXPERIMENTAL)
    return set_err(QLDPC_ENOTSUP, "engine 4 is built only with -DQLDPC_EXPERIMENTAL=1 (tools/build_variant.py)");
  r = Route();
  slot_var.clear();
  r.precision = precision;
  r.engine = ((want_engine >= 1 && want_engine <= 4) || want_engine == 6) ? want_engine : 3;
  if ((g->max_col > 8 || min_col_slots > 8) && r.engine != 6) {
    if (r.engine == 1) return set_err(QLDPC_ENOTSUP, "column degree > 8");
    r.engine = 6;
  }
  const int colmax = std::max(g->max_col, min_col_slots);
  r.DMAX = colmax <= 4 ? 4 : 8;
  if (r.engine == 3 && precision == 32 && colmax > 4 && colmax <= 6 && env_int("QLDPC_E3_D56", 1) != 0) r.DMAX = colmax;
  if (r.engine == 3 && precision == 64 && colmax == 5 && env_int("QLDPC_E3_D56", 1) != 0) r.DMAX = 5;
  if (r.engine == 6) return to_hbm(g, r, slot_var);
  const int tsize = precision == 32 ? 4 : 8;
  if (r.engine == 1) {
    const int rc = choose_geometry(g->n, g->m, vars_per_thread, max_spill_free_vpl(precision, r.DMAX), r.TB, r.VPL);
    if (rc) return rc;
    r.lds_bytes = (int)lds_for(precision, g->m);
    return get_variant(precision, r.VPL, r.DMAX).dec_k ? 0 : set_err(QLDPC_ENOTSUP, "no kernel variant");
  }
  if (r.engine == 4 && g->max_row > 8) r.engine = 3;
  r.nch = r.engine == 4 ? 8 * tsize / 16 : (std::max(1, g->max_row) * tsize + 15) / 16;
  if (route_vslots(r, g->m) >= 0xFFFF)
    return to_hbm(g, r, slot_var, "V image exceeds 65535 message slots (QLDPC_HBM_FALLBACK=0)");
  const int pref = r.DMAX == 4 ? kPrefVplR : 4;
  int vmax = r.DMAX == 4 ? kMaxVplR : 5;
  Route big = r;
  big.ea_shift = 2;
  if (r.engine == 3 && precision == 32 && r.DMAX == 4 && !fits(r, g) && fits(big, g) && env_int("QLDPC_E3_BIG", 1) != 0) r = big;
  admit_tail(g, vars_per_thread, r);
  admit_m2s(g, uniform, vars_per_thread, r);
  admit_m2st(g, uniform, vars_per_thread, r);
  admit_d5_256(g, r, pref, vars_per_thread, vmax);
  admit_m2s8(g, uniform, pref, vmax, vars_per_thread, r);
  if (r.engine >= 3 && ((r.DMAX != 4 && !(r.engine == 3 && (r.DMAX == 5 || r.DMAX == 6))) ||
                        (!r.fb && choose_rgeometry(g->n, g->m, vars_per_thread, r.TB, r.VPL, pref, vmax)) || !fits(r, g) ||
                        (precision == 64 && r.DMAX == 5 && !r.m2s && !use_f64w(r)))) {
    r.ea_shift = r.tail = r.m2s = r.vslots_dummy = r.m2s_pk = r.fb = 0;
    r.engine = 2;
    r.nch = (std::max(1, g->max_row) * tsize + 15) / 16;
    if (r.DMAX == 5 || r.DMAX == 6) r.DMAX = 8;
  }
  const int vslots = route_vslots(r, g->m);
  if (r.engine >= 3) {
    r.NS = 1;
    r.lds_bytes = (int)route_lds(r, vslots, g->m);
  } else {
    const int rc = choose_sgeometry(g->n, g->m, vars_per_thread, r.TB, r.VPL);
    if (rc) return rc;
    const int img = (int)slot_img_bytes(vslots, g->m, tsize);
    r.NS = choose_ns(img);
    r.lds_bytes = (int)slot_lds_bytes(r.NS, img, kChunkMax);
    const int bpc = std::max(1, kLdsMax / std::max(1, r.lds_bytes));
    if (vars_per_thread <= 0 && env_int("QLDPC_TB", 0) <= 0 && bpc * r.TB / 64 < 16) {
      const int tb = std::min(kMaxThreadsS, round_up((16 + bpc - 1) / bpc * 64, 64));
      if (tb > r.TB) {
        r.TB = tb;
        r.VPL = (g->n + tb - 1) / tb;
      }
    }
  }
  if (r.lds_bytes > kLdsMax) return to_hbm(g, r, slot_var, "per-shot LDS image exceeds 160 KiB (QLDPC_HBM_FALLBACK=0)");
  const bool sort3 = r.engine == 3 && r.DMAX >= 4 && env_int("QLDPC_DEGSORT", 1) != 0;
  const bool sort2 = sort3 && (r.fb || (r.tail && precision == 64 && (!r.m2s || r.nch == 4))) && env_int("QLDPC_D2K", 1) != 0;
  if (r.engine == 3 && precision == 64 && r.tail && r.m2s == 1 && r.nch == 4) {
    slot_var = st_plan(g, r.TB, r.VPL, r.DMAX, env_int("QLDPC_NW", 1) != 0, env_int("QLDPC_NW_BAL", 1) != 0).slots;
  } else {
    slot_var = sort2 ? degree_sorted(g, {2, 3}) : sort3 ? degree_sorted(g, {3}) : degree_sorted(g, {});
    slot_var.resize((size_t)r.VPL * r.TB, -1);
  }
  r.d3k = sort3 ? leading_slots(g, slot_var, r.TB, r.VPL, 3) : 0;
  r.d2k = sort2 ? leading_slots(g, slot_var, r.TB, r.VPL, 2) : 0;
  if (precision != 32 && !use_f64w(r) && !use_f64x(r) && !r.tail && !r.m2s) r.d3k = 0;
  if (slot_variant(r).dec_k) return 0;
  return (r.engine == 3 || r.engine == 4) ? to_hbm(g, r, slot_var, "no kernel variant") : set_err(QLDPC_ENOTSUP, "no kernel variant");
}

struct HostTables {
  std::vector<uint32_t> edges;
  std::vector<int> lab;
  std::vector<uint8_t> rdeg;
  std::vector<uint32_t> rowtab;
};

static void m2v_lane_search(const qldpc_graph* g, const Route& r, std::vector<int32_t>& slot_var) {
  const int TBm = r.TB, VPLm = r.VPL, DM = r.DMAX, M = g->m;
  const int ng = (M + 31) / 32;
  std::vector<int> L((size_t)ng * 32, 0);
  std::vector<int> C((size_t)VPLm * DM * (TBm / 32) * 32, 0);
  auto cidx = [&](int k, int d, int h, int b) { return (((size_t)k * DM + d) * (TBm / 32) + h) * 32 + b; };
  auto add = [&](int j, int pos, int sg) {
    const int k = pos / TBm, t = pos % TBm, b = t % 32, h = t / 32;
    const auto& rows = g->col_rows[j];
    for (int d = 0; d < (int)rows.size(); ++d) {
      L[(size_t)(rows[d] / 32) * 32 + b] += sg;
      C[cidx(k, d, h, (rows[d] + 1) % 32)] += sg;
    }
  };
  auto sq = [&](int j, int pos) {
    const int k = pos / TBm, t = pos % TBm, b = t % 32, h = t / 32;
    long long v = 0;
    const auto& rows = g->col_rows[j];
    for (int d = 0; d < (int)rows.size(); ++d) v += 2 * L[(size_t)(rows[d] / 32) * 32 + b] + C[cidx(k, d, h, (rows[d] + 1) % 32)];
    return v;
  };
  for (int pos = 0; pos < VPLm * TBm; ++pos)
    if (slot_var[pos] >= 0) add(slot_var[pos], pos, +1);
  uint64_t rs = 0xD1B54A32D192ED03ull;
  auto rnd = [&]() { rs ^= rs << 13; rs ^= rs >> 7; rs ^= rs << 17; return rs; };
  const int iters = env_int("QLDPC_M2V_PERM_IT", 400000);
  for (int it = 0; it < iters; ++it) {
    const int k = (int)(rnd() % (uint64_t)VPLm);
    const int pa = k * TBm + (int)(rnd() % (uint64_t)TBm), pb = k * TBm + (int)(rnd() % (uint64_t)TBm);
    const int ja = slot_var[pa], jb = slot_var[pb];
    if (ja < 0 || jb < 0 || pa == pb || (pa % 32) == (pb % 32) && (pa / 32) == (pb / 32)) continue;
    if (g->col_rows[ja].size() != g->col_rows[jb].size()) continue;
    add(ja, pa, -1);
    add(jb, pb, -1);
    const long long before = sq(ja, pa) + sq(jb, pb);
    const long long after = sq(ja, pb) + sq(jb, pa);
    if (after <= before) {
// ... 3 lines not shown
      add(ja, pb, +1);
    } else {
      add(ja, pa, +1);
      add(jb, pb, +1);
    }
  }
}

static int m2v_row_table(const qldpc_graph* g, const Route& r, const std::vector<int32_t>& slot_var,
                         std::vector<uint32_t>& tab) {
  const int TBm = r.TB, VPLm = r.VPL, d3 = std::min(r.d3k, VPLm);
  auto ecnt = [&](int k) { return 3 * std::min(k, d3) + 4 * std::max(0, k - d3); };
  if (ecnt(VPLm - 1) * TBm != r.m2v_vlast) return set_err(QLDPC_ENOTSUP, "m2v layout mismatch");
  const uint32_t sent = (uint32_t)(r.vslots_m2v - 1) * 8u;
  std::vector<std::vector<uint32_t>> roff(g->m);
  for (int k = 0; k < VPLm; ++k)
    for (int t = 0; t < TBm; ++t) {
      const int j = slot_var[(size_t)k * TBm + t];
      if (j < 0) continue;
      const auto& rows = g->col_rows[j];
      for (int d = 0; d < (int)rows.size(); ++d) {
        const int vs = k < VPLm - 1 ? (ecnt(k) + d) * TBm + t : r.m2v_vlast + d * r.m2v_nl + t;
        roff[rows[d]].push_back((uint32_t)vs * 8u);
      }
    }
  for (int i = 0; i < g->m; ++i) {
    if (roff[i].size() > 7) return set_err(QLDPC_ENOTSUP, "m2v row wider than 7");
    while (roff[i].size() < 8) roff[i].push_back(sent);
  }
  if (env_int("QLDPC_M2V_ORDER", 1) != 0) {
    uint64_t rs = 0x9E3779B97F4A7C15ull;
    auto rnd = [&]() { rs ^= rs << 13; rs ^= rs >> 7; rs ^= rs << 17; return rs; };
    for (int q = 0; q < 4; ++q)
      for (int g0 = 0; g0 < TBm; g0 += 32) {
        std::vector<int> rr;
        for (int l = 0; l < 32; ++l)
          if (q * TBm + g0 + l < g->m) rr.push_back(q * TBm + g0 + l);
        if (rr.size() < 2) continue;
        int cnt[7][32] = {{0}};
        auto bk = [&](uint32_t o) { return (int)((o / 8u) % 32u); };
        for (int i : rr)
          for (int e = 0; e < 7; ++e)
            if (roff[i][e] != sent) cnt[e][bk(roff[i][e])]++;
        for (int it = 0; it < 4000; ++it) {
          const int i = rr[rnd() % rr.size()], a = (int)(rnd() % 7), b = (int)(rnd() % 7);
          const uint32_t oa = roff[i][a], ob = roff[i][b];
          if (a == b || oa == ob) continue;
          auto term = [&](int e, uint32_t o, int dlt) {
            if (o == sent) return 0;
            const int c = cnt[e][bk(o)];
            return dlt > 0 ? 2 * c + 1 : -(2 * c - 1);
          };
          int d = term(a, oa, -1);
          if (oa != sent) cnt[a][bk(oa)]--;
          d += term(b, ob, -1);
          if (ob != sent) cnt[b][bk(ob)]--;
          d += term(a, ob, +1);
          if (ob != sent) cnt[a][bk(ob)]++;
          d += term(b, oa, +1);
          if (oa != sent) cnt[b][bk(oa)]++;
          if (d <= 0) {
            roff[i][a] = ob;
            roff[i][b] = oa;
          } else {
            if (ob != sent) cnt[a][bk(ob)]--;
            if (oa != sent) cnt[b][bk(oa)]--;
            if (oa != sent) cnt[a][bk(oa)]++;
            if (ob != sent) cnt[b][bk(ob)]++;
          }
        }
      }
  }
  tab.assign((size_t)4 * TBm * 4, 0);
  for (int q = 0; q < 4; ++q)
    for (int t = 0; t < TBm; ++t) {
      const int i = q * TBm + t;
      uint32_t o[8];
      for (int e = 0; e < 8; ++e) o[e] = i < g->m ? roff[i][e] : sent;
      for (int w = 0; w < 4; ++w) tab[((size_t)q * TBm + t) * 4 + w] = o[2 * w] | (o[2 * w + 1] << 16);
    }
  return 0;
}

static int build_tables(qldpc_bp* bp, HostTables& T) {
  const qldpc_graph* g = bp->g;
  const Route& r = bp->route;
  if (r.engine == 1) {
    const int TB = r.TB, VPL = r.VPL, DM = r.DMAX, D2 = DM / 2;
    T.edges.assign((size_t)VPL * D2 * TB, 0xFFFFFFFFu);
    for (int k = 0; k < VPL; ++k)
      for (int t = 0; t < TB; ++t) {
        const int j = k * TB + t;
        if (j >= g->n) continue;
        const auto& rows = g->col_rows[j];
        for (int d = 0; d < DM; ++d) {
          const uint32_t v = d < (int)rows.size() ? (uint32_t)rows[d] : 0xFFFFu;
          uint32_t& w = T.edges[((size_t)k * D2 + d / 2) * TB + t];
          w = (d & 1) ? ((w & 0xFFFFu) | (v << 16)) : ((w & 0xFFFF0000u) | v);
        }
      }
    return 0;
  }
  const int tsize = r.precision == 32 ? 4 : 8;
  const RLayout L = route_layout(r, route_vslots(r, g->m), g->m);
  if (r.m2s == 3 && env_int("QLDPC_M2V_PERM", 0) != 0) m2v_lane_search(g, r, bp->slot_var);
  if (r.engine == 3 && env_int("QLDPC_LABEL", r.precision == 64 && !r.m2s ? 1 : 0) != 0)
    T.lab = label_checks(g, r, bp->slot_var, &bp->gather_conf[0], &bp->gather_conf[1]);
  const bool f64e3 = r.engine == 3 && r.precision == 64 && r.m2s != 3;
  int ndummy = 0;
  build_slot_edges(g, r, bp->slot_var, T.edges, (r.engine == 3 && env_int("QLDPC_BANKOPT", 1) != 0) ? (int)(L.v / 4) : -1,
                   T.lab, r.m2s == 1 && env_int("QLDPC_M2S_PLACE", 1) != 0,
                   r.vslots_dummy ? (1 + g->m * r.nch) * (16 / tsize) : -1, &ndummy,
                   !f64e3 ? 0 : (r.m2s || r.tail) ? 1 : env_int("QLDPC_ANNEAL_2W", 1) != 0 ? 2 : 0, -1,
                   (r.tail && r.vslots_dummy) ? (int)(L.t - L.v) / tsize : -1);
  if (ndummy != r.vslots_dummy) return set_err(QLDPC_EINVAL, "m2s private dummy slot count mismatch");
  if (f64e3 && r.ea_shift == 0) lds_model_var_phase(T.edges, r, L.v, bp->lds_model);
  if (r.m2s == 3)
    if (const int rc = m2v_row_table(g, r, bp->slot_var, T.rowtab)) return rc;
  if (r.engine >= 3) {
    T.rdeg.resize(std::max(1, g->m));
    for (int i = 0; i < g->m; ++i) T.rdeg[T.lab.empty() ? i : T.lab[i]] = (uint8_t)(g->row_ptr[i + 1] - g->row_ptr[i]);
  }
  return 0;
}

static int upload(DevBuf& buf, const void* src, size_t bytes, const char* what) {
  if (const int rc = buf.alloc(std::max<size_t>(bytes, 1))) return rc;
  if (bytes && hipMemcpy(buf.p, src, bytes, hipMemcpyHostToDevice) != hipSuccess) return set_err(QLDPC_EHIP, what);
  return 0;
}

static int create_min_sum(qldpc_graph* g, const double* channel_probs, int32_t max_iter, int32_t bp_method,
                          double ms_scaling_factor, int32_t precision, int32_t vars_per_thread,
                          int32_t min_col_slots, int forced_engine, qldpc_bp** out) {
  if (!out) return set_err(QLDPC_EINVAL, "NULL argument");
  int rc = validate_create(g, channel_probs, precision, bp_method);
  if (rc) return rc;
  QLDPC_HIP(hipSetDevice(g->device));
  if (bp_method == QLDPC_PRODUCT_SUM) return create_ps(g, channel_probs, max_iter, precision, out);
  auto* bp = new qldpc_bp();
  auto fail = [&](int code) {
    qldpc_bp_destroy(bp);
    return code;
  };
  bp->g = g;
  bp->max_iter = max_iter > 0 ? max_iter : g->n;
  bp->method = bp_method;
  bp->alpha = ms_scaling_factor;
  bp->probs.assign(channel_probs, channel_probs + g->n);
  if ((rc = plan_route(g, !QLDPC_M2S_UNIL || uniform_priors(channel_probs, g->n), precision, vars_per_thread,
                       min_col_slots, forced_engine, bp->route, bp->slot_var)))
    return fail(rc);
  const Route& r = bp->route;
  const int tsize = precision == 32 ? 4 : 8;
  const void* kern;
  if (r.engine == 6) {
    if ((rc = hbm_prepare(bp)) || (rc = bp->llr.alloc((size_t)g->n * tsize))) return fail(rc);
    kern = hbm_kernel(precision);
  } else {
    HostTables T;
    if ((rc = build_tables(bp, T))) return fail(rc);
    bp->npos = g->n;
    if (!T.lab.empty()) {
      std::vector<int32_t> inv(g->m);
      for (int i = 0; i < g->m; ++i) inv[T.lab[i]] = i;
      if ((rc = upload(bp->rperm, inv.data(), inv.size() * 4, "upload check labels"))) return fail(rc);
    }
    if ((r.m2s == 3 && (rc = upload(bp->rowtab, T.rowtab.data(), T.rowtab.size() * 4, "upload m2v row table"))) ||
        (r.engine >= 3 && (rc = upload(bp->rdeg, T.rdeg.data(), T.rdeg.size(), "upload row degrees"))) ||
        (rc = upload(bp->vchk, T.edges.data(), T.edges.size() * 4, "upload edge table")) ||
        (!bp->slot_var.empty() && (rc = upload(bp->perm, bp->slot_var.data(), bp->slot_var.size() * 4, "upload slot map"))) ||
        (rc = bp->llr.alloc((size_t)r.VPL * r.TB * tsize)))
      return fail(rc);
    kern = r.engine == 1 ? get_variant(precision, r.VPL, r.DMAX).dec_k : slot_variant(r).dec_k;
  }
  if ((rc = upload_llr(bp))) return fail(rc);
  int nb = 0;
  if (hipOccupancyMaxActiveBlocksPerMultiprocessor(&nb, kern, r.TB, r.lds_bytes) != hipSuccess) nb = 1;
  bp->blocks_per_cu = std::max(1, nb);
  if ((rc = device_cus(g->device, bp->cus))) return fail(rc);
  bp1_prepare(bp);
  *out = bp;
  return 0;
}

int qldpc_bp_plan(const qldpc_graph* g, const double* channel_probs, int32_t bp_method, int32_t precision,
                  int32_t vars_per_thread, int32_t min_col_slots, int32_t* out, int32_t out_len) {
  if (!out || out_len < 8) return set_err(QLDPC_EINVAL, "out needs 8 entries");
  int rc = validate_create(g, channel_probs, precision, bp_method);
  if (rc) return rc;
  if (bp_method == QLDPC_PRODUCT_SUM) return set_err(QLDPC_ENOTSUP, "the product-sum geometry needs the device");
  Route r;
  std::vector<int32_t> slot_var;
  if ((rc = plan_route(g, !QLDPC_M2S_UNIL || uniform_priors(channel_probs, g->n), precision, vars_per_thread,
                       min_col_slots, 0, r, slot_var)))
    return rc;
  const int32_t v[8] = {r.engine, route_kernel_id(r), r.nch, r.TB, r.VPL, r.lds_bytes, r.engine == 3 ? r.d3k : 0,
// ... 77 lines not shown
  *out = bp;
  return 0;
}

int qldpc_bp_create_serial(qldpc_graph* g, const double* channel_probs, int32_t max_iter, double ms_scaling_factor,
                           int32_t precision, int32_t soft, qldpc_bp** out) {
  if (!out) return set_err(QLDPC_EINVAL, "NULL argument");
  int rc = validate_create(g, channel_probs, precision, QLDPC_MIN_SUM);
  if (rc) return rc;
  if ((rc = serial_check_params(g->n, max_iter, precision))) return rc;
  QLDPC_HIP(hipSetDevice(g->device));
  auto* bp = new qldpc_bp();
  auto fail = [&](int code) {
    qldpc_bp_destroy(bp);
    return code;
  };
  bp->g = g;
  bp->route.engine = 8;
  bp->route.precision = precision;
  bp->method = QLDPC_MIN_SUM;
  bp->alpha = ms_scaling_factor;
  bp->max_iter = max_iter;
  bp->probs.assign(channel_probs, channel_probs + g->n);
  bp->bp1_off = true;
  bp->sr_soft = soft != 0;
  if ((rc = upload_csr_csc(bp)) || (rc = bp->llr.alloc(std::max<size_t>(1, g->n) * (precision == 32 ? 4 : 8))) ||
      (rc = upload_llr(bp)) || (rc = device_cus(g->device, bp->cus)) ||
      (rc = serial_prepare(bp, env_int("QLDPC_SERIAL_WS", 0) == 1, env_int("QLDPC_SERIAL_IDX", 1) != 0,
                           env_int("QLDPC_SERIAL_TB", 0), kLdsMax)))
    return fail(rc);
  *out = bp;
  return 0;
}

int qldpc_bp_set_channel_probs(qldpc_bp* bp, const double* channel_probs) {
  if (!bp || !channel_probs) return set_err(QLDPC_EINVAL, "NULL argument");
  if (bp->route.m2s && QLDPC_M2S_UNIL && !uniform_priors(channel_probs, bp->g->n))
    return set_err(QLDPC_ENOTSUP, "this decoder's kernels hold one uniform prior: create a new decoder for "
                                  "non-uniform channel_probs");
  bp->probs.assign(channel_probs, channel_probs + bp->g->n);
  const int rc = upload_llr(bp);
  if (rc) return rc;
  bp1_prepare(bp);
  return 0;
}

int qldpc_bp_degree3_slots(const qldpc_bp* bp, int32_t* d3k) {
  if (!bp || !d3k) return set_err(QLDPC_EINVAL, "NULL argument");
  *d3k = bp->route.engine == 3 ? bp->route.d3k : 0;
  return 0;
}

int qldpc_bp_lds_model(const qldpc_bp* bp, int64_t* out6) {
  if (!bp || !out6) return set_err(QLDPC_EINVAL, "NULL argument");
  for (int q = 0; q < 6; ++q) out6[q] = bp->lds_model[q];
  return 0;
}

int qldpc_m2s_place_model(const qldpc_graph* g, int32_t anneal_iters, int64_t* out6) {
  if (!g || !out6) return set_err(QLDPC_EINVAL, "NULL argument");
  int n3 = 0;
  for (int j = 0; j < g->n; ++j) {
    const int d = (int)g->col_rows[j].size();
    if (d != 3 && d != 4) return set_err(QLDPC_ENOTSUP, "m2s placement model: column degrees 3 / 4 only");
    n3 += d == 3;
  }
  Route r;
  r.engine = 3;
  r.tail = r.m2s = 1;
  r.nch = 3;
  if (g->max_row < 1 || g->max_row > 7 || choose_rgeometry(g->n, g->m, 0, r.TB, r.VPL) || r.TB > 256 || r.VPL < 4 ||
      r.VPL > 8 || !(n3 % r.TB == 0 || n3 == g->n))
    return set_err(QLDPC_ENOTSUP, "graph outside the m2s envelope (rows <= 7, <= 256 threads x 4-8 slots)");
  std::vector<int32_t> slot_var = degree_sorted(g, {3});
  slot_var.resize((size_t)r.VPL * r.TB, -1);
  r.d3k = leading_slots(g, slot_var, r.TB, r.VPL, 3);
  const uint32_t vbase = route_layout(r, route_vslots(r, g->m), g->m).v;
  std::vector<uint32_t> edges;
  build_slot_edges(g, r, slot_var, edges, (int)(vbase / 4), {}, 1, -1, nullptr, 1, anneal_iters);
  lds_model_var_phase(edges, r, vbase, out6);
  return 0;
}

int qldpc_bp_bank_stats(const qldpc_bp* bp, int32_t* before, int32_t* after) {
  if (!bp) return set_err(QLDPC_EINVAL, "NULL decoder");
  if (before) *before = bp->gather_conf[0];
  if (after) *after = bp->gather_conf[1];
  return 0;
}

int qldpc_bp_kernel_id(const qldpc_bp* bp, int32_t* kernel_id, int32_t* row_chunks) {
  if (!bp) return set_err(QLDPC_EINVAL, "NULL decoder");
  if (kernel_id) *kernel_id = route_kernel_id(bp->route);
  if (row_chunks) *row_chunks = bp->route.nch;
  return 0;
}

int qldpc_bp_engine(const qldpc_bp* bp, int32_t* engine) {
  if (!bp || !engine) return set_err(QLDPC_EINVAL, "NULL argument");
  *engine = bp->route.engine;
  return 0;
}

int qldpc_bp_geometry(const qldpc_bp* bp, int32_t* threads, int32_t* vpl, int32_t* lds_bytes,
                      int32_t* blocks_per_cu) {
  if (!bp) return set_err(QLDPC_EINVAL, "NULL decoder");
  if (threads) *threads = bp->route.TB;
  if (vpl) *vpl = bp->route.VPL;
  if (lds_bytes) *lds_bytes = bp->route.lds_bytes;
  if (blocks_per_cu) *blocks_per_cu = bp->blocks_per_cu;
  return 0;
}

static SectorDev sector_of(const qldpc_bp* bp, const unsigned long long* lmask, int kw) {
  SectorDev s;
  s.vchk = static_cast<const uint32_t*>(bp->vchk.p);
  s.llr = bp->llr.p;
  s.lmask = lmask;
  s.m = bp->g->m;
  s.n = bp->g->n;
  s.kw = kw;
  s.max_iter = bp->max_iter;
  s.alpha = bp->alpha;
  return s;
}

static SSector ssector_of(const qldpc_bp* bp, const unsigned long long* lmask, int kw) {
  SSector s;
  s.edges = static_cast<const uint32_t*>(bp->vchk.p);
  s.llr = bp->llr.p;
  s.lmask = lmask;
  s.rdeg = static_cast<const uint8_t*>(bp->rdeg.p);
  s.perm = static_cast<const int32_t*>(bp->perm.p);
  s.rperm = static_cast<const int32_t*>(bp->rperm.p);
  s.d3k = bp->route.d3k;
  s.m = bp->g->m;
  s.n = bp->g->n;
  s.kw = kw;
  s.max_iter = bp->max_iter;
  s.nch = bp->route.nch;
  s.vpl = bp->route.VPL;
  s.alpha = bp->alpha;
  s.rows = static_cast<const uint32_t*>(bp->rowtab.p);
  s.vlast = bp->route.m2v_vlast;
  s.vnl = bp->route.m2v_nl;
  s.npos = bp->npos > 0 ? bp->npos : bp->g->n;
  s.nw = bp->route.nw;
  s.live_last = bp->route.live_last;
  return s;
}

static int chunk_for(long long count, long long grid, int ns) {
  long long c = (count + grid - 1) / grid;
  c = std::max<long long>(c, ns);
  c = std::min<long long>(c, kChunkMax);
  return (int)c;
}

static int decode_batch(qldpc_bp* bp, const uint8_t* d_synd, uint8_t* d_corr, int32_t* d_iters, uint8_t* d_conv,
                        double* d_post, int64_t B, void* stream);

int qldpc_bp_decode_batch(qldpc_bp* bp, const uint8_t* d_synd, uint8_t* d_corr, int32_t* d_iters, uint8_t* d_conv,
                          int64_t B, void* stream) {
  return decode_batch(bp, d_synd, d_corr, d_iters, d_conv, nullptr, B, stream);
}

// ... 39 lines not shown
    a.B = B;
    a.mmax = bp->g->m;
    a.vslots = route_vslots(bp->route, bp->g->m);
    a.img_bytes = (int)slot_img_bytes(a.vslots, a.mmax, tsize);
    a.chunk = chunk_for(B, cap, bp->route.NS);
    a.work = nullptr;
#if QLDPC_STAMPS
    a.stamps = debug_stamps_buffer();
#else
    a.stamps = nullptr;
#endif
    if (bp->route.engine >= 3 && env_int("QLDPC_DYN", 1) != 0) {
      if (!bp->work.p && bp->work.alloc(16)) return QLDPC_ENOMEM;
      constexpr long long kMaxQueuePops = 8192;
      a.chunk = (int)std::max<long long>(1, std::min<long long>(kChunkMax, B / (cap * std::max(1, env_int("QLDPC_DYN_PER", 64)))));
      a.chunk = (int)std::min<long long>(kChunkMax, std::max<long long>(a.chunk, (B + kMaxQueuePops - 1) / kMaxQueuePops));
      QLDPC_HIP(hipMemsetAsync(bp->work.p, 0, 4, (hipStream_t)stream));
      a.work = static_cast<unsigned int*>(bp->work.p);
    }
    const long long nchunks = (B + a.chunk - 1) / a.chunk;
    const int grid = (int)std::max<long long>(1, std::min<long long>(nchunks, cap));
    SVariant v = slot_variant(bp->route);
    QLDPC_HIP(v.dec(dim3(grid), dim3(bp->route.TB), bp->route.lds_bytes, (hipStream_t)stream, a));
  }
  return 0;
}

static int build_lmask(const qldpc_graph* L, int n, DevBuf& buf, int& kw) {
  if (!L) {
    kw = 0;
    return 0;
  }
  if (L->n != n) return set_err(QLDPC_EINVAL, "logical operator width != code length");
  kw = (L->m + 63) / 64;
  if (kw > 4) return set_err(QLDPC_ENOTSUP, "more than 256 logical operators");
  if (kw == 0) kw = 1;
  std::vector<unsigned long long> mask((size_t)n * kw, 0ull);
  for (int r = 0; r < L->m; ++r)
    for (int e = L->row_ptr[r]; e < L->row_ptr[r + 1]; ++e)
      mask[(size_t)L->col_idx[e] * kw + r / 64] |= 1ull << (r % 64);
  int rc = buf.alloc(mask.size() * 8);
  if (rc) return rc;
  QLDPC_HIP(hipMemcpy(buf.p, mask.data(), mask.size() * 8, hipMemcpyHostToDevice));
  return 0;
}

static int mc_create_staged(qldpc_bp* dec_x, const qldpc_graph* logical_x, qldpc_bp* dec_z,
                            const qldpc_graph* logical_z, qldpc_mc** out) {
  qldpc_bp* d0 = dec_x ? dec_x : dec_z;
  if (dec_x && dec_z && (dec_x->g->n != dec_z->g->n || dec_x->g->device != dec_z->g->device))
    return set_err(QLDPC_EINVAL, "sector decoders differ in code length or device");
  QLDPC_HIP(hipSetDevice(d0->g->device));
  auto* mc = new qldpc_mc();
  mc->dec[0] = dec_x;
  mc->dec[1] = dec_z;
  mc->route = d0->route;
  int rc = mc->counters.alloc(sizeof(qldpc_counters));
  if (!rc) rc = staged_mc_prepare(mc, logical_x, logical_z);
  if (rc) {
    staged_mc_release(mc);
    mc->counters.release();
    delete mc;
    return rc;
  }
  *out = mc;
  return 0;
}

int qldpc_mc_create_staged(qldpc_bp* dec_x, const qldpc_graph* logical_x, qldpc_bp* dec_z,
                           const qldpc_graph* logical_z, qldpc_mc** out) {
  if (!out || (!dec_x && !dec_z)) return set_err(QLDPC_EINVAL, "need at least one sector decoder");
  return mc_create_staged(dec_x, logical_x, dec_z, logical_z, out);
}

int qldpc_mc_create(qldpc_bp* dec_x, const qldpc_graph* logical_x, qldpc_bp* dec_z, const qldpc_graph* logical_z,
                    qldpc_mc** out) {
  if (!out || (!dec_x && !dec_z)) return set_err(QLDPC_EINVAL, "need at least one sector decoder");
  qldpc_bp* d0 = dec_x ? dec_x : dec_z;
  const bool staged = (dec_x && dec_x->route.engine >= 5) || (dec_z && dec_z->route.engine >= 5) ||
                      (dec_x && dec_x->route.tail && (!dec_x->route.m2s || dec_x->route.nch == 4)) ||
                      (dec_z && dec_z->route.tail && (!dec_z->route.m2s || dec_z->route.nch == 4)) ||
                      (dec_x && dec_z &&
                       (dec_x->route.m2s != dec_z->route.m2s || dec_x->route.tail != dec_z->route.tail || dec_x->route.fb != dec_z->route.fb ||
                        dec_x->route.m2s_pk != dec_z->route.m2s_pk)) ||
                      (dec_x && dec_z && dec_x->route.m2s && dec_x->route.d3k != dec_z->route.d3k) ||
                      env_int("QLDPC_MC_STAGED", 0) == 1;
  if (staged) return mc_create_staged(dec_x, logical_x, dec_z, logical_z, out);
  if (dec_x && dec_z) {
    if (dec_x->g->n != dec_z->g->n) return set_err(QLDPC_EINVAL, "sector code lengths differ");
    if (dec_x->route.TB != dec_z->route.TB || dec_x->route.VPL != dec_z->route.VPL || dec_x->route.DMAX != dec_z->route.DMAX ||
        dec_x->route.precision != dec_z->route.precision || dec_x->route.engine != dec_z->route.engine)
      return set_err(QLDPC_EINVAL, "sector decoders need identical geometry/precision (same vars_per_thread)");
    if (dec_x->g->device != dec_z->g->device) return set_err(QLDPC_EINVAL, "sector decoders on different devices");
    if (dec_x->route.m2s != dec_z->route.m2s || dec_x->route.tail != dec_z->route.tail || dec_x->route.fb != dec_z->route.fb)
      return set_err(QLDPC_EINVAL, "sector decoders use different LDS layouts (QLDPC_M2S)");
  }
  QLDPC_HIP(hipSetDevice(d0->g->device));
  auto* mc = new qldpc_mc();
  auto fail = [&](int code) {
    mc->lmask[0].release();
    mc->lmask[1].release();
    mc->counters.release();
    mc->work.release();
    delete mc;
    return code;
  };
  mc->dec[0] = dec_x;
  mc->dec[1] = dec_z;
  int rc = 0;
  if (dec_x && (rc = build_lmask(logical_x, dec_x->g->n, mc->lmask[0], mc->kw[0]))) return fail(rc);
  if (dec_z && (rc = build_lmask(logical_z, dec_z->g->n, mc->lmask[1], mc->kw[1]))) return fail(rc);
  mc->route = d0->route;
  if (dec_x && dec_z && dec_x->route.ea_shift != dec_z->route.ea_shift)
    return fail(set_err(QLDPC_EINVAL, "sector decoders use different LDS address scales"));
  mc->route.d3k = std::min(dec_x ? dec_x->route.d3k : 1 << 20, dec_z ? dec_z->route.d3k : 1 << 20);
  mc->route.d2k = 0;
  if (dec_x && dec_z && dec_x->route.nch != dec_z->route.nch) mc->route.nch = 0;
  mc->mmax = std::max(dec_x ? dec_x->g->m : 0, dec_z ? dec_z->g->m : 0);
  const void* kern;
  if (mc->route.engine == 1) {
    mc->route.lds_bytes = (int)lds_for(mc->route.precision, mc->mmax);
    kern = get_variant(mc->route.precision, mc->route.VPL, mc->route.DMAX).mc_k;
  } else {
    const int tsize = mc->route.precision == 32 ? 4 : 8;
    for (qldpc_bp* d : {dec_x, dec_z})
      if (d)
        mc->vslots = std::max(mc->vslots, route_vslots(d->route, d->g->m));
    mc->img_bytes = (int)slot_img_bytes(mc->vslots, mc->mmax, tsize);
    if (mc->route.engine >= 3) {
      if (!route_fits(mc->route, mc->vslots, mc->mmax))
        return fail(set_err(QLDPC_ENOTSUP, "sector images exceed the register engines' 64 KiB addressing (QLDPC_ENGINE=2)"));
      mc->route.NS = 1;
      mc->route.lds_bytes = (int)route_lds(mc->route, mc->vslots, mc->mmax);
    } else {
      mc->route.NS = choose_ns(mc->img_bytes);
      mc->route.lds_bytes = (int)slot_lds_bytes(mc->route.NS, mc->img_bytes, kChunkMax);
    }
    kern = slot_variant(mc->route).mc_k;
  }
  if (mc->route.lds_bytes > kLdsMax) return fail(set_err(QLDPC_ENOTSUP, "per-shot LDS image exceeds 160 KiB"));
  if (!kern) return fail(set_err(QLDPC_ENOTSUP, "no kernel variant"));
  int nb = 0;
  if (hipOccupancyMaxActiveBlocksPerMultiprocessor(&nb, kern, mc->route.TB, mc->route.lds_bytes) != hipSuccess) nb = 1;
  mc->blocks_per_cu = std::max(1, nb);
  mc->cus = d0->cus;
  if ((rc = mc->counters.alloc(sizeof(qldpc_counters))) || (rc = mc->work.alloc(16))) return fail(rc);
  *out = mc;
  return 0;
}

int qldpc_mc_set_osd(qldpc_mc* mc, qldpc_osd_gpu* osd_x, qldpc_osd_gpu* osd_z) {
  if (!mc) return set_err(QLDPC_EINVAL, "NULL mc");
  qldpc_osd_gpu* o[2] = {osd_x, osd_z};
  for (int q = 0; q < 2; ++q) {
    if (!o[q]) continue;
    if (mc->staged || mc->route.engine != 3)
      return set_err(QLDPC_ENOTSUP, "BP+OSD shot loop needs the fused engine-3 MC kernel");
    if (!mc->dec[q] || !osd_gpu_matches(o[q], mc->dec[q]->g))
      return set_err(QLDPC_EINVAL, q == 0 ? "X-sector OSD handle was built on a different graph than dec_x"
                                          : "Z-sector OSD handle was built on a different graph than dec_z");
  }
  mc->osd[0] = osd_x;
  mc->osd[1] = osd_z;
  mc->c_cap = 0;
  return 0;
}

// ... 41 lines not shown
  }
  QLDPC_HIP(hipSetDevice((mc->dec[0] ? mc->dec[0] : mc->dec[1])->g->device));
  const bool bposd = mc->route.engine != 1 && ((need[0] && mc->osd[0]) || (need[1] && mc->osd[1]));
  if (bposd) {
    long long slot_bytes = 0;
    for (int q = 0; q < 2; ++q)
      if (need[q] && mc->osd[q]) {
        const long long n = mc->dec[q]->g->n, m = mc->dec[q]->g->m;
        slot_bytes = std::max(slot_bytes, n * 8 + m + n + 8 + n);
      }
    const long long budget = (long long)std::max(1, env_int("QLDPC_OSD_CAPTURE_MB", 2048)) << 20;
    const long long slots = std::max<long long>(1024, budget / slot_bytes);
    if (shot_count > slots) {
      const long long n = (mc->dec[0] ? mc->dec[0] : mc->dec[1])->g->n;
      for (long long off = 0; off < shot_count; off += slots) {
        const long long c = std::min(slots, shot_count - off);
        int rc = qldpc_mc_launch(mc, px, py, pz, seed, shot_begin + (uint64_t)off, c, logical_mode,
                                 d_uniforms ? d_uniforms + off * n : nullptr, d_counters, d_fail ? d_fail + off : nullptr,
                                 d_err ? d_err + off * n : nullptr, d_corr ? d_corr + off * 2 * n : nullptr,
                                 d_iters ? d_iters + off * 2 : nullptr, grid_blocks, stream);
        if (rc) return rc;
      }
      return 0;
    }
  }
  const long long cap = (long long)mc->blocks_per_cu * mc->cus;
  const double t1 = pz, t2 = pz + px, t3 = (pz + px) + py;
  if (mc->route.engine == 1) {
    McArgs a;
    std::memset(&a, 0, sizeof(a));
    for (int q = 0; q < 2; ++q) {
      if (!need[q]) continue;
      a.sec[a.nsec] = sector_of(mc->dec[q], static_cast<const unsigned long long*>(mc->lmask[q].p), mc->kw[q]);
      a.sec_id[a.nsec++] = q;
    }
    a.logical_mode = logical_mode;
    a.mmax = mc->mmax;
    a.t1 = t1; a.t2 = t2; a.t3 = t3;
    a.K1 = ceil_2p53(t1); a.K2 = ceil_2p53(t2); a.K3 = ceil_2p53(t3);
    a.seed = seed; a.shot_begin = shot_begin; a.shot_count = shot_count;
    a.uniforms = d_uniforms;
    a.counters = static_cast<unsigned long long*>(d_counters);
    a.fail = d_fail; a.err = d_err; a.corr = d_corr; a.iters = d_iters;
    long long grid = grid_blocks > 0 ? grid_blocks : cap;
    grid = std::max<long long>(1, std::min<long long>(grid, shot_count));
    Variant v = get_variant(mc->route.precision, mc->route.VPL, mc->route.DMAX);
    QLDPC_HIP(v.mc(dim3((unsigned)grid), dim3(mc->route.TB), mc->route.lds_bytes, (hipStream_t)stream, a));
  } else {
    SMcArgs a;
    std::memset(&a, 0, sizeof(a));
    int ids[2] = {0, 0};
    for (int q = 0; q < 2; ++q) {
      if (!need[q]) continue;
      a.sec[a.nsec] = ssector_of(mc->dec[q], static_cast<const unsigned long long*>(mc->lmask[q].p), mc->kw[q]);
      ids[a.nsec++] = q;
    }
    a.sec_id0 = ids[0];
    a.sec_id1 = ids[1];
    a.logical_mode = logical_mode;
    a.mmax = mc->mmax;
    a.vslots = mc->vslots;
    a.img_bytes = mc->img_bytes;
    const long long want = grid_blocks > 0 ? grid_blocks : cap;
    a.chunk = chunk_for(shot_count, want, mc->route.NS);
    if (mc->route.engine >= 3 && mc->work.p && env_int("QLDPC_DYN", 1) != 0) {
      const int per = std::max(1, env_int("QLDPC_DYN_PER", 64));
      a.chunk = (int)std::max<long long>(1, std::min<long long>(kChunkMax, shot_count / (want * per)));
      QLDPC_HIP(hipMemsetAsync(mc->work.p, 0, 4, (hipStream_t)stream));
      a.work = static_cast<unsigned int*>(mc->work.p);
    }
    a.t1 = t1; a.t2 = t2; a.t3 = t3;
    a.K1 = ceil_2p53(t1); a.K2 = ceil_2p53(t2); a.K3 = ceil_2p53(t3);
    a.seed = seed; a.shot_begin = shot_begin; a.shot_count = shot_count;
    a.uniforms = d_uniforms;
    a.counters = static_cast<unsigned long long*>(d_counters);
    a.fail = d_fail; a.err = d_err; a.corr = d_corr; a.iters = d_iters;
#if QLDPC_STAMPS
    a.stamps = debug_stamps_buffer();
#endif
    const long long nchunks = (shot_count + a.chunk - 1) / a.chunk;
    if (nchunks > 0x7fffffffLL) return set_err(QLDPC_EINVAL, "too many shots for one launch (chunk count >= 2^31)");
    const long long grid = std::max<long long>(1, std::min<long long>(nchunks, want));
    a.cls_cache = nullptr;
    const size_t cc_need = (size_t)grid * (size_t)a.chunk * (size_t)mc->route.TB * 2;
    if (a.nsec == 2 && !d_uniforms && mc->route.VPL <= 8 && env_int("QLDPC_CLS_CACHE", 1) != 0 && cc_need <= (256u << 20)) {
      const size_t need = cc_need;
      if (mc->cls_cache.bytes < need) {
        mc->cls_cache.release();
        int rc = mc->cls_cache.alloc(need);
        if (rc) return rc;
      }
      a.cls_cache = static_cast<uint16_t*>(mc->cls_cache.p);
    }
    hipStream_t st = (hipStream_t)stream;
    if (bposd) {
      if (mc->c_cap < shot_count) {
        for (int q = 0; q < 2; ++q) {
          for (DevBuf* d : {&mc->c_post[q], &mc->c_synd[q], &mc->c_err[q], &mc->c_shot[q], &mc->c_outw[q]}) d->release();
          if (!mc->dec[q] || !mc->osd[q]) continue;
          const int n = mc->dec[q]->g->n, m = mc->dec[q]->g->m;
          int rc;
          if ((rc = mc->c_post[q].alloc((size_t)shot_count * n * 8)) || (rc = mc->c_synd[q].alloc((size_t)shot_count * m)) ||
              (rc = mc->c_err[q].alloc((size_t)shot_count * n)) || (rc = mc->c_shot[q].alloc((size_t)shot_count * 8)) ||
              (rc = mc->c_outw[q].alloc((size_t)shot_count * n)))
            return rc;
        }
        mc->c_fail.release();
        int rc;
        if ((rc = mc->c_fail.alloc((size_t)shot_count)) || (!mc->c_n.p && (rc = mc->c_n.alloc(16)))) return rc;
        mc->c_cap = shot_count;
      }
      QLDPC_HIP(hipMemsetAsync(mc->c_n.p, 0, 16, st));
      a.c_n = static_cast<unsigned int*>(mc->c_n.p);
      a.c_cap = shot_count;
      for (int q = 0; q < 2; ++q) {
        const bool on = need[q] && mc->osd[q];
        a.c_post[q] = on ? static_cast<double*>(mc->c_post[q].p) : nullptr;
        a.c_synd[q] = on ? static_cast<uint8_t*>(mc->c_synd[q].p) : nullptr;
        a.c_err[q] = on ? static_cast<uint8_t*>(mc->c_err[q].p) : nullptr;
        a.c_shot[q] = on ? static_cast<long long*>(mc->c_shot[q].p) : nullptr;
      }
      if (!a.fail) a.fail = static_cast<uint8_t*>(mc->c_fail.p);
    }
    SVariant v = slot_variant(mc->route);
    QLDPC_HIP(v.mc(dim3((unsigned)grid), dim3(mc->route.TB), mc->route.lds_bytes, st, a));
    if (bposd) {
      unsigned int nc[4] = {0, 0, 0, 0};
      QLDPC_HIP(hipMemcpyAsync(nc, mc->c_n.p, 16, hipMemcpyDeviceToHost, st));
      QLDPC_HIP(hipStreamSynchronize(st));
      for (int q = 0; q < 2; ++q) {
        if (!(need[q] && mc->osd[q]) || nc[q] == 0) continue;
        if ((long long)nc[q] > a.c_cap)
          return set_err(QLDPC_EINVAL, "BP+OSD capture overflow: more candidates than capture slots");
        const long long ncand = nc[q];
        int rc = osd_gpu_bposd_stage(mc->osd[q], static_cast<const uint8_t*>(mc->c_synd[q].p),
                                     static_cast<const double*>(mc->c_post[q].p), static_cast<const uint8_t*>(mc->c_err[q].p),
                                     static_cast<const long long*>(mc->c_shot[q].p), static_cast<uint8_t*>(mc->c_outw[q].p),
                                     ncand, static_cast<const unsigned long long*>(mc->lmask[q].p), mc->kw[q], q,
                                     logical_mode, a.fail, static_cast<unsigned long long*>(d_counters), st);
        if (rc) return rc;
      }
    }
  }
  return 0;
}

int qldpc_mc_launch_weight(qldpc_mc* mc, int32_t weight, double px, double py, double pz, uint64_t seed,
                           uint64_t shot_begin, int64_t shot_count, int32_t logical_mode, void* d_counters,
                           uint8_t* d_fail, uint8_t* d_err, uint8_t* d_corr, int32_t* d_iters, void* stream) {
  if (!mc || !d_counters) return set_err(QLDPC_EINVAL, "NULL argument");
  if (logical_mode < 0 || logical_mode > 2) return set_err(QLDPC_EINVAL, "logical_mode must be 0 (X), 1 (Z), 2 (Total)");
  if (!mc->staged)
    return set_err(QLDPC_ENOTSUP, "fixed-weight shots need a staged handle (qldpc_mc_create_staged)");
  if (mc->osd[0] || mc->osd[1]) return set_err(QLDPC_ENOTSUP, "fixed-weight shots do not run the BP+OSD stage");
  const qldpc_bp* d0 = mc->dec[0] ? mc->dec[0] : mc->dec[1];
  StagedWeight fw;
  fw.weight = weight;
  if (int rc = weight_thresholds(weight, d0->g->n, px, py, pz, &fw.K1, &fw.K2)) return rc;
  if (shot_count <= 0) return 0;
  const bool need[2] = {logical_mode != 1, logical_mode != 0};
  for (int q = 0; q < 2; ++q)
    if (need[q] && !mc->dec[q])
      return set_err(QLDPC_EINVAL, q == 0 ? "logical_mode needs the X sector (hz decoder)"
                                          : "logical_mode needs the Z sector (hx decoder)");
  QLDPC_HIP(hipSetDevice(d0->g->device));
  return staged_mc_launch(mc, px, py, pz, seed, shot_begin, shot_count, logical_mode, nullptr, d_counters, d_fail,
                          d_err, d_corr, d_iters, (hipStream_t)stream, &fw);
}

int qldpc_mc_run(qldpc_mc* mc, double px, double py, double pz, uint64_t seed, uint64_t shot_begin,
                 int64_t shot_count, int32_t logical_mode, qldpc_counters* out, void* stream) {
  if (!mc || !out) return set_err(QLDPC_EINVAL, "NULL argument");
  hipStream_t s = (hipStream_t)stream;
  QLDPC_HIP(hipMemsetAsync(mc->counters.p, 0, sizeof(qldpc_counters), s));
  int rc = qldpc_mc_launch(mc, px, py, pz, seed, shot_begin, shot_count, logical_mode, nullptr, mc->counters.p,
// ... 19 lines not shown
```

### qldpc_fault_tolerance_amd/csrc/route.h

```cpp
#pragma once
#include <cstdint>

namespace qldpc_rt {

constexpr int kHbmThreads = 256;
constexpr int kHbmMaxDeg = 12;

struct Route {
  int engine = 2, precision = 64;
  int DMAX = 4, TB = 64, VPL = 1, NS = 1;
  int nch = 0;
  int d3k = 0;
  int d2k = 0;
  int ea_shift = 0;
  int tail = 0;
  int m2s = 0;
  int fb = 0;
  int m2s_pk = 0;
  int vslots_dummy = 0;
  int vslots_m2v = 0;
  int m2v_vlast = 0, m2v_nl = 0;
  uint32_t nw = 0;
  uint32_t live_last = 0;
  int lds_bytes = 0;
};

inline int route_vslots(const Route& r, int m) {
  return r.vslots_m2v ? r.vslots_m2v : (1 + m * r.nch) * (r.precision == 32 ? 4 : 2) + r.vslots_dummy;
}

}
```

### qldpc_fault_tolerance_amd/csrc/variants.h

```cpp
#pragma once
#include "bp_reg.h"

#ifndef QLDPC_EXPERIMENTAL
#define QLDPC_EXPERIMENTAL 0
#endif

namespace qldpc {

using DecLaunch = hipError_t (*)(dim3, dim3, size_t, hipStream_t, const DecArgs&);
using McLaunch = hipError_t (*)(dim3, dim3, size_t, hipStream_t, const McArgs&);
using SDecLaunch = hipError_t (*)(dim3, dim3, size_t, hipStream_t, const SDecArgs&);
using SMcLaunch = hipError_t (*)(dim3, dim3, size_t, hipStream_t, const SMcArgs&);

struct Variant {
  DecLaunch dec;
  McLaunch mc;
  const void* dec_k;
  const void* mc_k;
};

struct SVariant {
  SDecLaunch dec;
  SMcLaunch mc;
  const void* dec_k;
  const void* mc_k;
};

Variant get_variant_f32_d4(int vpl);
Variant get_variant_f32_d8(int vpl);
Variant get_variant_f64_d4(int vpl);
Variant get_variant_f64_d8(int vpl);
SVariant get_rvariant_f32(int vpl, int d3k);
SVariant get_rvariant_f32_a(int vpl, int d3k);
SVariant get_rvariant_f32_b(int vpl, int d3k);
SVariant get_rvariant_f32_c(int vpl, int d3k);
SVariant get_rvariant_f32_big(int vpl, int d3k);
SVariant get_rvariant_f32_d5(int vpl, int d3k);
SVariant get_rvariant_f32_d6(int vpl, int d3k);
SVariant get_rvariant_f64(int vpl);
SVariant get_rvariant_f32_w(int vpl, int d3k);
SVariant get_rvariant_f64_w(int vpl, int d3k, int nch);
SVariant get_rvariant_f64_w3(int vpl, int d3k);
SVariant get_rvariant_f64_w_d5(int vpl, int d3k, int nch);
SVariant get_rvariant_f64_x(int vpl, int d3k);
SVariant get_rvariant_f64_w4(int vpl, int d3k);
SVariant get_rvariant_f64_st(int vpl, int d3k, int d2k = 0);
SVariant get_rvariant_f64_st_hi(int vpl, int d3k);
SVariant get_rvariant_f32_st(int vpl, int d3k);
SVariant get_rvariant_f64_m2st(int vpl, int d3k, int d2k);
SVariant get_rvariant_f64_m2s(int vpl, int d3k);
SVariant get_rvariant_f64_m2s8(int vpl, int d3k);
SVariant get_rvariant_f64_m2s8pk(int vpl, int d3k);
SVariant get_rvariant_f64_m2v(int vpl, int d3k);
SVariant get_rvariant_f64_c2s(int vpl, int d3k);
SVariant get_rvariant_f32_stfb(int vpl, int d3k, int d2k);
SVariant get_r4variant_f32(int vpl);
SVariant get_r4variant_f64(int vpl);
SVariant get_r4variant_f64_w(int vpl);
SVariant get_svariant_f32_d4(int ns);
SVariant get_svariant_f32_d8(int ns);
SVariant get_svariant_f64_d4(int ns);
SVariant get_svariant_f64_d8(int ns);

#ifdef QLDPC_VARIANT_TU
template <typename T, int VPL, int DMAX>
hipError_t launch_dec(dim3 g, dim3 b, size_t lds, hipStream_t s, const DecArgs& a) {
  hipLaunchKernelGGL((bp_decode_kernel<T, VPL, DMAX>), g, b, lds, s, a);
  return hipGetLastError();
}
template <typename T, int VPL, int DMAX>
hipError_t launch_mc(dim3 g, dim3 b, size_t lds, hipStream_t s, const McArgs& a) {
  hipLaunchKernelGGL((mc_kernel<T, VPL, DMAX>), g, b, lds, s, a);
  return hipGetLastError();
}
template <typename T, int VPL, int DMAX>
Variant make_variant() {
  return Variant{&launch_dec<T, VPL, DMAX>, &launch_mc<T, VPL, DMAX>,
                 reinterpret_cast<const void*>(&bp_decode_kernel<T, VPL, DMAX>),
                 reinterpret_cast<const void*>(&mc_kernel<T, VPL, DMAX>)};
}
template <typename T, int DMAX>
Variant pick_vpl(int vpl) {
  switch (vpl) {
    case 1: return make_variant<T, 1, DMAX>();
    case 2: return make_variant<T, 2, DMAX>();
    case 3: return make_variant<T, 3, DMAX>();
    case 4: return make_variant<T, 4, DMAX>();
    case 5: return make_variant<T, 5, DMAX>();
    case 6: return make_variant<T, 6, DMAX>();
    case 7: return make_variant<T, 7, DMAX>();
    case 8: return make_variant<T, 8, DMAX>();
    case 10: return make_variant<T, 10, DMAX>();
    case 12: return make_variant<T, 12, DMAX>();
    default: return Variant{nullptr, nullptr, nullptr, nullptr};
  }
}

template <typename T, int DMAX, int NS>
hipError_t slaunch_dec(dim3 g, dim3 b, size_t lds, hipStream_t s, const SDecArgs& a) {
  hipLaunchKernelGGL((sdec_kernel<T, DMAX, NS>), g, b, lds, s, a);
  return hipGetLastError();
}
template <typename T, int DMAX, int NS>
hipError_t slaunch_mc(dim3 g, dim3 b, size_t lds, hipStream_t s, const SMcArgs& a) {
  hipLaunchKernelGGL((smc_kernel<T, DMAX, NS>), g, b, lds, s, a);
  return hipGetLastError();
}
template <typename T, int DMAX, int NS>
SVariant make_svariant() {
  return SVariant{&slaunch_dec<T, DMAX, NS>, &slaunch_mc<T, DMAX, NS>,
                  reinterpret_cast<const void*>(&sdec_kernel<T, DMAX, NS>),
                  reinterpret_cast<const void*>(&smc_kernel<T, DMAX, NS>)};
}
template <typename T, int DMAX>
SVariant pick_sns(int ns) {
  switch (ns) {
    case 1: return make_svariant<T, DMAX, 1>();
    case 2: return make_svariant<T, DMAX, 2>();
    case 4: return make_svariant<T, DMAX, 4>();
    default: return SVariant{nullptr, nullptr, nullptr, nullptr};
  }
}

template <typename T, int VPL, int ENG, int D3K, int DM = 4, int LB = kMaxThreadsS, int NCH = 0>
hipError_t rlaunch_dec(dim3 g, dim3 b, size_t lds, hipStream_t s, const SDecArgs& a) {
  hipLaunchKernelGGL((rdec_kernel<T, DM, VPL, ENG, D3K, LB, NCH>), g, b, lds, s, a);
  return hipGetLastError();
}
template <typename T, int VPL, int ENG, int D3K, int DM = 4, int LB = kMaxThreadsS, int NCH = 0>
hipError_t rlaunch_mc(dim3 g, dim3 b, size_t lds, hipStream_t s, const SMcArgs& a) {
  hipLaunchKernelGGL((rmc_kernel<T, DM, VPL, ENG, D3K, LB, NCH>), g, b, lds, s, a);
  return hipGetLastError();
}
// ... 38 lines not shown
```

Measured before the change: 1.276 million.

## Add position-major m2s LDS layout engine with annealed check placement

```diff
diff --git a/include/qldpc_hip.h b/include/qldpc_hip.h
--- a/include/qldpc_hip.h
+++ b/include/qldpc_hip.h
@@ -161,6 +161,8 @@
 
 int qldpc_bp_lds_model(const qldpc_bp *bp, int64_t *out6);
 int qldpc_m2s_place_model(const qldpc_graph *g, int32_t anneal_iters, int64_t *out6);
+int qldpc_m2s_pm_place(const qldpc_graph *g, int32_t anneal_iters, int32_t *geom4, int32_t *lab, int32_t *slot_var,
+                       int32_t slot_cap, uint32_t *edges, int32_t edge_cap, int64_t *out6);
 int qldpc_bp_bank_stats(const qldpc_bp *bp, int32_t *before, int32_t *after);
 
 #define QLDPC_COMM_ID_BYTES 128
diff --git a/qldpc_fault_tolerance_amd/_native.py b/qldpc_fault_tolerance_amd/_native.py
--- a/qldpc_fault_tolerance_amd/_native.py
+++ b/qldpc_fault_tolerance_amd/_native.py
@@ -21,7 +21,7 @@
     "qldpc_comm_allreduce_counters_group", "qldpc_comm_destroy", "qldpc_mc_run_sharded", "qldpc_sample_errors",
     "qldpc_stream_sync", "qldpc_bp_kernel_id", "qldpc_build_flags", "qldpc_circ_create", "qldpc_circ_set_final_osd", "qldpc_circ_set_sampler",
     "qldpc_circ_info", "qldpc_circ_launch", "qldpc_circ_sample", "qldpc_circ_destroy",
-    "qldpc_shard_range", "qldpc_bp_lds_model", "qldpc_m2s_place_model", "qldpc_bp_plan",
+    "qldpc_shard_range", "qldpc_bp_lds_model", "qldpc_m2s_place_model", "qldpc_m2s_pm_place", "qldpc_bp_plan",
     "qldpc_circ_create_single_shot", "qldpc_circ_set_round_firstmin",
     "qldpc_dist_create", "qldpc_dist_run_host", "qldpc_dist_run", "qldpc_dist_geometry", "qldpc_dist_destroy",
     "qldpc_mc_create_staged", "qldpc_mc_launch_weight", "qldpc_sample_errors_weight",
@@ -201,6 +201,8 @@
     L.qldpc_bp_lds_model.argtypes = [_vp, ctypes.POINTER(_i64)]
     L.qldpc_m2s_place_model.restype = ctypes.c_int
     L.qldpc_m2s_place_model.argtypes = [_vp, ctypes.c_int32, ctypes.POINTER(_i64)]
+    L.qldpc_m2s_pm_place.restype = ctypes.c_int
+    L.qldpc_m2s_pm_place.argtypes = [_vp, _i32, _vp, _vp, _vp, _i32, _vp, _i32, ctypes.POINTER(_i64)]
     L.qldpc_shard_range.restype = ctypes.c_int
     L.qldpc_shard_range.argtypes = [_i64, _i32, _i32, ctypes.POINTER(_i64), ctypes.POINTER(_i64)]
     L.qldpc_circ_destroy.restype = ctypes.c_int
diff --git a/qldpc_fault_tolerance_amd/csrc/bp_reg.h b/qldpc_fault_tolerance_amd/csrc/bp_reg.h
--- a/qldpc_fault_tolerance_amd/csrc/bp_reg.h
+++ b/qldpc_fault_tolerance_amd/csrc/bp_reg.h
@@ -56,7 +56,10 @@
 constexpr int eng_sh(int E) { return (E / 10) % 10 ? 2 : 0; }
 constexpr bool eng_kv64(int E) { return (E / 100) % 10 != 0; }
 constexpr int eng_tail(int E) { return (E / 1000) % 10; }
-constexpr bool eng_m2s(int E) { return (E / 10000) % 10 == 1 || (E / 10000) % 10 == 4; }
+constexpr bool eng_m2s(int E) { return (E / 10000) % 10 == 1 || (E / 10000) % 10 == 4 || (E / 10000) % 10 == 5; }
+constexpr bool eng_pm(int E) { return (E / 10000) % 10 == 5; }
+constexpr int kPmPlane = 256, kPmRows = 7;
+__host__ __device__ constexpr int pm_vslots(int rpt) { return 2 + kPmRows * kPmPlane * rpt; }
 constexpr bool eng_m2v(int E) { return (E / 10000) % 10 == 4; }
 template <int D3K>
 __host__ __device__ constexpr int m2v_ecnt(int k) { return 3 * (k < D3K ? k : D3K) + 4 * (k > D3K ? k - D3K : 0); }
@@ -1045,6 +1048,71 @@
   return mism;
 }
 
+template <typename T, bool FIRST, int RPT>
+__device__ inline int pm_check(unsigned char* smem, const RLayout& Ly, int m, int wtid, int TB, uint32_t& sbits) {
+  using U = typename FT<T>::U;
+  static_assert(sizeof(T) == 8, "m2s: fp64 only");
+  constexpr uint32_t PS = (uint32_t)(kPmPlane * RPT) * 8u;
+  int mism = 0;
+  int q = 0;
+  int tid = wtid;
+  asm volatile("" : "+v"(tid));
+  const uint32_t sb = lds_base(smem);
+  uint32_t rb = sb + Ly.v + 16u + (uint32_t)tid * 8u;
+  uint32_t fp = sb + Ly.f + 4u * (uint32_t)(tid + 1);
+  uint32_t cp = sb + (uint32_t)(tid + 1) * 8u;
+  const uint32_t drb = (uint32_t)TB * 8u, dfp = 4u * (uint32_t)TB;
+  for (int i = tid; i < m; i += TB, ++q) {
+    asm volatile("" : "+v"(rb));
+    const uint32_t rp = rb & 0xFFFFu;
+    double x[kPmRows];
+#pragma unroll
+    for (int p = 0; p < kPmRows; ++p) {
+      using W = typename LdsWord<8>::type;
+      const W w = *(LdsPtr<const volatile W>)(uintptr_t)(rp + (uint32_t)p * PS);
+      __builtin_memcpy(&x[p], &w, 8);
+    }
+    const uint32_t fcur = lds_ld<uint32_t, true>(nullptr, fp);
+    uint32_t s;
+    if (FIRST) {
+      s = ((fcur >> 1) ^ (fcur >> 2)) & 1u;
+      sbits |= s << q;
+      lds_st<uint32_t, true>(nullptr, fp, (fcur & 4u) | ((fcur >> 2) & 1u));
+    } else {
+      s = (sbits >> q) & 1u;
+      mism |= (int)((fcur ^ s) & 1u);
+    }
+    double f1 = FT<T>::val(FT<T>::kSent), f2 = f1;
+    uint32_t px = s ? 0x80000000u : 0u;
+    uint32_t apos = 0u;
+#pragma unroll
+    for (int p = 0; p < kPmRows; ++p) {
+      apos = __builtin_fabs(x[p]) < f1 ? (uint32_t)p : apos;
+      double t;
+      asm("v_max_f64 %0, %1, |%2|" : "=v"(t) : "v"(f1), "v"(x[p]));
+      asm("v_min_f64 %0, %1, %2" : "=v"(f2) : "v"(f2), "v"(t));
+      asm("v_min_f64 %0, %1, |%2|" : "=v"(f1) : "v"(f1), "v"(x[p]));
+    }
+#pragma unroll
+    for (int p = 0; p + 1 < kPmRows; p += 2) {
+      uint32_t pp;
+      asm("v_bitop3_b32 %0, %1, %2, %3 bitop3:0x96"
+          : "=v"(pp)
+          : "v"(px), "v"((uint32_t)(FT<T>::bits(x[p]) >> 32)), "v"((uint32_t)(FT<T>::bits(x[p + 1]) >> 32)));
+      px = pp;
+    }
+    px ^= (uint32_t)(FT<T>::bits(x[kPmRows - 1]) >> 32);
+    const U par = (U)(px & 0x80000000u) << 32;
+    lds_st<U, true>(nullptr, cp, FT<T>::bits(f1) | par);
+    asm("" : "+v"(apos));
+    lds_st<U, true>(nullptr, rp + apos * PS, FT<T>::bits(f2) | par);
+    rb += drb;
+    fp += dfp;
+    cp += drb;
+  }
+  return mism;
+}
+
 template <typename T, bool FIRST>
 __device__ inline int m2v_check(unsigned char* smem, const RLayout& Ly, int m, int tid, int TB, uint32_t& sbits,
                                 const M2vRows& RW, uint32_t vbase) {
@@ -1415,13 +1483,16 @@
         int jv[VPL];
 #pragma unroll
         for (int k = 0; k < VPL; ++k) jv[k] = S.perm[k * TB + tidl];
-        uint16_t* cc = nullptr;
+        uint8_t* cc = nullptr;
         bool cc_read = false;
-        uint32_t cw = 0;
-        if (A->cls_cache && !A->uniforms && VPL <= 8) {
-          cc = A->cls_cache + ((long long)blockIdx.x * A->chunk + sh) * TB + tidl;
+        uint32_t cv[VPL] = {};
+        if (A->cls_cache && !A->uniforms) {
+          cc = A->cls_cache + ((long long)blockIdx.x * A->chunk + sh) * (long long)n;
           cc_read = q == A->sec_id1;
-          if (cc_read) cw = *cc;
+          if (cc_read) {
+#pragma unroll
+            for (int k = 0; k < VPL; ++k) cv[k] = jv[k] >= 0 ? cc[jv[k]] : 0u;
+          }
         }
 #pragma unroll
         for (int k = 0; k < VPL; ++k) {
@@ -1432,11 +1503,11 @@
               const double u = A->uniforms[sl * (long long)n + j];
               cls = (u < A->t1) ? 2u : (A->t1 <= u && u < A->t2) ? 1u : (A->t2 <= u && u < A->t3) ? 3u : 0u;
             } else if (cc_read) {
-              cls = (cw >> (2 * k)) & 3u;
+              cls = cv[k];
             } else {
               const unsigned long long kk = philox_k53(A->seed, gshot, (uint32_t)j);
               cls = (kk < A->K1) ? 2u : (kk < A->K2) ? 1u : (kk < A->K3) ? 3u : 0u;
-              cw |= cls << (2 * k);
+              if (cc) cc[j] = (uint8_t)cls;
             }
             const uint32_t e = (q == 0) ? (cls & 1u) : (cls >> 1);
             eb |= e << k;
@@ -1455,7 +1526,6 @@
             }
           }
         }
-        if (cc && !cc_read) *cc = (uint16_t)cw;
       } else {
         const uint8_t* srow = D->synd + (c0 + sh) * (long long)m;
         for (int i = tidl; i < m; i += TB) {
@@ -1510,6 +1580,8 @@
       c2s_check<T, true, NCH, eng_tail(ENG)>(smem, Ly, m, tid, TB, sb, adaptive ? (T)0.5 : alpha_fixed);
     else if constexpr (eng_m2v(ENG))
       m2v_check<T, true>(smem, Ly, m, tid, TB, sb, rwv, sbase + Ly.v);
+    else if constexpr (eng_pm(ENG))
+      pm_check<T, true, NCH>(smem, Ly, m, tid, TB, sb);
     else if constexpr (eng_m2s(ENG))
       m_check<T, true, NCH, eng_tail(ENG)>(smem, Ly, m, wbase, tid, TB, sb);
     else if constexpr (NCH > 0)
@@ -1574,6 +1646,8 @@
           mism = c2s_check<T, false, NCH, eng_tail(ENG)>(smem, Ly, m, tid, TB, sb, alpha_next);
         else if constexpr (eng_m2v(ENG))
           mism = m2v_check<T, false>(smem, Ly, m, tid, TB, sb, rwv, sbase + Ly.v);
+        else if constexpr (eng_pm(ENG))
+          mism = pm_check<T, false, NCH>(smem, Ly, m, tid, TB, sb);
         else if constexpr (eng_m2s(ENG))
           mism = m_check<T, false, NCH, eng_tail(ENG)>(smem, Ly, m, wbase, tid, TB, sb);
         else if constexpr (NCH > 0)
diff --git a/qldpc_fault_tolerance_amd/csrc/bp_slot.h b/qldpc_fault_tolerance_amd/csrc/bp_slot.h
--- a/qldpc_fault_tolerance_amd/csrc/bp_slot.h
+++ b/qldpc_fault_tolerance_amd/csrc/bp_slot.h
@@ -48,7 +48,7 @@
   long long* c_shot[2];
   long long c_cap;
   unsigned long long* stamps;
-  uint16_t* cls_cache;
+  uint8_t* cls_cache;
 };
 
 struct SDecArgs {
diff --git a/qldpc_fault_tolerance_amd/csrc/kern_r_f64_m2sp1.hip b/qldpc_fault_tolerance_amd/csrc/kern_r_f64_m2sp1.hip
--- /dev/null
+++ b/qldpc_fault_tolerance_amd/csrc/kern_r_f64_m2sp1.hip
@@ -0,0 +1,15 @@
+#define QLDPC_VARIANT_TU 1
+#include "variants.h"
+
+namespace qldpc {
+SVariant get_rvariant_f64_m2sp1(int vpl, int d3k) {
+  switch (vpl) {
+    case 4: return pick_rd3k<double, 4, 50103, 4, 256, 1>(d3k);
+    case 5: return pick_rd3k<double, 5, 50103, 4, 256, 1>(d3k);
+    case 6: return pick_rd3k<double, 6, 50103, 4, 256, 1>(d3k);
+    case 7: return pick_rd3k<double, 7, 50103, 4, 256, 1>(d3k);
+    case 8: return pick_rd3k<double, 8, 50103, 4, 256, 1>(d3k);
+    default: return SVariant{nullptr, nullptr, nullptr, nullptr};
+  }
+}
+}
diff --git a/qldpc_fault_tolerance_amd/csrc/kern_r_f64_m2sp2.hip b/qldpc_fault_tolerance_amd/csrc/kern_r_f64_m2sp2.hip
--- /dev/null
+++ b/qldpc_fault_tolerance_amd/csrc/kern_r_f64_m2sp2.hip
@@ -0,0 +1,15 @@
+#define QLDPC_VARIANT_TU 1
+#include "variants.h"
+
+namespace qldpc {
+SVariant get_rvariant_f64_m2sp2(int vpl, int d3k) {
+  switch (vpl) {
+    case 4: return pick_rd3k<double, 4, 50103, 4, 256, 2>(d3k);
+    case 5: return pick_rd3k<double, 5, 50103, 4, 256, 2>(d3k);
+    case 6: return pick_rd3k<double, 6, 50103, 4, 256, 2>(d3k);
+    case 7: return pick_rd3k<double, 7, 50103, 4, 256, 2>(d3k);
+    case 8: return pick_rd3k<double, 8, 50103, 4, 256, 2>(d3k);
+    default: return SVariant{nullptr, nullptr, nullptr, nullptr};
+  }
+}
+}
diff --git a/qldpc_fault_tolerance_amd/csrc/kern_r_f64_m2sp3.hip b/qldpc_fault_tolerance_amd/csrc/kern_r_f64_m2sp3.hip
--- /dev/null
+++ b/qldpc_fault_tolerance_amd/csrc/kern_r_f64_m2sp3.hip
@@ -0,0 +1,15 @@
+#define QLDPC_VARIANT_TU 1
+#include "variants.h"
+
+namespace qldpc {
+SVariant get_rvariant_f64_m2sp3(int vpl, int d3k) {
+  switch (vpl) {
+    case 4: return pick_rd3k<double, 4, 50103, 4, 256, 3>(d3k);
+    case 5: return pick_rd3k<double, 5, 50103, 4, 256, 3>(d3k);
+    case 6: return pick_rd3k<double, 6, 50103, 4, 256, 3>(d3k);
+    case 7: return pick_rd3k<double, 7, 50103, 4, 256, 3>(d3k);
+    case 8: return pick_rd3k<double, 8, 50103, 4, 256, 3>(d3k);
+    default: return SVariant{nullptr, nullptr, nullptr, nullptr};
+  }
+}
+}
diff --git a/qldpc_fault_tolerance_amd/csrc/qldpc_hip.hip b/qldpc_fault_tolerance_amd/csrc/qldpc_hip.hip
--- a/qldpc_fault_tolerance_amd/csrc/qldpc_hip.hip
+++ b/qldpc_fault_tolerance_amd/csrc/qldpc_hip.hip
@@ -92,6 +92,9 @@
     if (r.m2s == 3)
       return (e3 && f64 && r.DMAX == 4 && r.ea_shift == 0 && r.TB == 256) ? get_rvariant_f64_m2v(r.VPL, r.d3k) : none;
     if (!ok) return none;
+    if (r.m2s == 1 && r.pm)
+      return r.pm == 1 ? get_rvariant_f64_m2sp1(r.VPL, r.d3k) : r.pm == 2 ? get_rvariant_f64_m2sp2(r.VPL, r.d3k)
+             : r.pm == 3 ? get_rvariant_f64_m2sp3(r.VPL, r.d3k) : none;
     return r.m2s == 2 ? get_rvariant_f64_c2s(r.VPL, r.d3k) : get_rvariant_f64_m2s(r.VPL, r.d3k);
   }
   if (r.tail) {
@@ -198,7 +201,7 @@
 }
 
 RLayout route_layout(const Route& r, int vslots, int mmax) {
-  return r_layout(r.engine, vslots, mmax, r.precision == 32 ? 4 : 8, r.tail, r.m2s, r.fb);
+  return r_layout(r.engine, vslots, mmax, r.precision == 32 ? 4 : 8, r.pm ? 0 : r.tail, r.m2s, r.fb);
 }
 size_t route_lds(const Route& r, int vslots, int mmax) {
   return r_lds_bytes((int)route_layout(r, vslots, mmax).total, kChunkMax);
@@ -965,7 +968,7 @@
   r.TB = kHbmThreads;
   r.VPL = 1;
   r.lds_bytes = 0;
-  r.ea_shift = r.tail = r.m2s = r.fb = r.m2s_pk = r.vslots_dummy = r.d3k = r.d2k = 0;
+  r.ea_shift = r.tail = r.m2s = r.pm = r.fb = r.m2s_pk = r.vslots_dummy = r.d3k = r.d2k = 0;
   r.nw = r.live_last = 0;
   slot_var.clear();
   return 0;
@@ -1031,6 +1034,12 @@
   if (r.m2s == 1 && tb == 256 && g->m <= 4 * 256 && v.vslots_m2v * 8 < 65536 && QLDPC_EXPERIMENTAL &&
       env_int("QLDPC_M2V", 0) != 0 && fits(v, g))
     r = v;
+  Route p = r;
+  p.pm = (g->m + 255) / 256;
+  const int pm_mode = env_int("QLDPC_M2S_PM", 1);
+  if (r.m2s == 1 && p.pm <= 3 && pm_mode != 0 && fits(p, g) &&
+      (pm_mode == 2 || route_lds(p, route_vslots(p, g->m), g->m) <= route_lds(r, route_vslots(r, g->m), g->m)))
+    r = p;
 }
 
 static void admit_m2st(const qldpc_graph* g, bool uniform, int vars_per_thread, Route& r) {
@@ -1140,7 +1149,7 @@
   if (r.engine >= 3 && ((r.DMAX != 4 && !(r.engine == 3 && (r.DMAX == 5 || r.DMAX == 6))) ||
                         (!r.fb && choose_rgeometry(g->n, g->m, vars_per_thread, r.TB, r.VPL, pref, vmax)) || !fits(r, g) ||
                         (precision == 64 && r.DMAX == 5 && !r.m2s && !use_f64w(r)))) {
-    r.ea_shift = r.tail = r.m2s = r.vslots_dummy = r.m2s_pk = r.fb = 0;
+    r.ea_shift = r.tail = r.m2s = r.pm = r.vslots_dummy = r.m2s_pk = r.fb = 0;
     r.engine = 2;
     r.nch = (std::max(1, g->max_row) * tsize + 15) / 16;
     if (r.DMAX == 5 || r.DMAX == 6) r.DMAX = 8;
@@ -1310,6 +1319,218 @@
   return 0;
 }
 
+static void pm_place(const qldpc_graph* g, const Route& r, std::vector<int32_t>& slot_var, std::vector<int>& lab,
+                     int anneal_iters) {
+  const int TB = r.TB, VPL = r.VPL, DM = r.DMAX, m = g->m;
+  lab.clear();
+  const int iters_env = anneal_iters >= 0 ? anneal_iters : env_int("QLDPC_M2S_ANNEAL", -1);
+  const long long iters = iters_env >= 0 ? iters_env : std::min<long long>(800LL * g->nnz, 1LL << 24);
+  if (iters <= 0 || m < 2) return;
+  constexpr int wr = 4, ws = 1, wmax = 16, rot_every = 64;
+  constexpr size_t kMemo = 16;
+  static std::mutex memo_mu;
+  static std::map<uint64_t, std::pair<std::vector<int>, std::vector<int32_t>>> memo;
+  uint64_t key = 0xcbf29ce484222325ull;
+  auto mix = [&](uint64_t v) { key = (key ^ v) * 0x100000001b3ull; };
+  for (long long v : {(long long)m, (long long)g->n, (long long)TB, (long long)VPL, (long long)r.pm, iters})
+    mix((uint64_t)v);
+  for (int32_t v : slot_var) mix((uint64_t)(uint32_t)v);
+  for (int32_t v : g->row_ptr) mix((uint64_t)(uint32_t)v);
+  for (int32_t v : g->col_idx) mix((uint64_t)(uint32_t)v);
+  {
+    std::lock_guard<std::mutex> lk(memo_mu);
+    auto it = memo.find(key);
+    if (it != memo.end() && (int)it->second.first.size() == m && it->second.second.size() == slot_var.size()) {
+      lab = it->second.first;
+      slot_var = it->second.second;
+      return;
+    }
+  }
+  lab.resize(m);
+  for (int i = 0; i < m; ++i) lab[i] = i;
+  const int n32 = (TB + 31) / 32, n16 = (TB + 15) / 16;
+  struct Grp {
+    uint8_t cnt[32] = {0};
+    int16_t hist[66] = {0};
+    int mx = 0;
+  };
+  std::vector<Grp> G32((size_t)VPL * DM * n32), G16((size_t)VPL * DM * n16);
+  auto gadd = [&](Grp& G, int b) {
+    const int c = G.cnt[b]++;
+    G.hist[c]--, G.hist[c + 1]++;
+    const int m0 = std::max(G.mx, 1);
+    G.mx = std::max(G.mx, c + 1);
+    return (long long)wmax * (std::max(G.mx, 1) - m0) + 2 * c + 1;
+  };
+  auto gsub = [&](Grp& G, int b) {
+    const int c = G.cnt[b]--;
+    G.hist[c]--, G.hist[c - 1]++;
+    const int m0 = std::max(G.mx, 1);
+    while (G.mx > 0 && G.hist[G.mx] == 0) --G.mx;
+    return (long long)wmax * (std::max(G.mx, 1) - m0) - (2 * c - 1);
+  };
+  std::vector<int> posof(g->n, -1), real;
+  for (int p = 0; p < VPL * TB; ++p)
+    if (slot_var[p] >= 0) {
+      posof[slot_var[p]] = p;
+      real.push_back(p);
+    }
+  std::vector<std::vector<std::pair<int, int>>> cedges(m);
+  for (int j = 0; j < g->n; ++j)
+    for (int t = 0; t < (int)g->col_rows[j].size() && t < DM; ++t) cedges[g->col_rows[j][t]].emplace_back(j, t);
+  auto touch = [&](int p, int t, int l, int sg) {
+    const int k = p / TB, ln = p % TB;
+    Grp& a = G32[(size_t)(k * DM + t) * n32 + ln / 32];
+    Grp& b = G16[(size_t)(k * DM + t) * n16 + ln / 16];
+    return sg > 0 ? wr * gadd(a, l & 31) + ws * gadd(b, l & 15) : wr * gsub(a, l & 31) + ws * gsub(b, l & 15);
+  };
+  auto var_at = [&](int j, int p, int sg) {
+    long long d = 0;
+    const auto& rows = g->col_rows[j];
+    for (int t = 0; t < (int)rows.size() && t < DM; ++t) d += touch(p, t, lab[rows[t]], sg);
+    return d;
+  };
+  auto check_as = [&](int i, int l, int sg) {
+    long long d = 0;
+    for (const auto& e : cedges[i])
+      if (posof[e.first] >= 0) d += touch(posof[e.first], e.second, l, sg);
+    return d;
+  };
+  auto fill = [&](int sg) {
+    long long c = 0;
+    for (int p : real) c += var_at(slot_var[p], p, sg);
+    return c;
+  };
+  {
+    std::vector<int32_t> sv2(slot_var);
+    int sc = 0;
+    for (size_t a0 = 0; a0 < real.size();) {
+      size_t a1 = a0;
+      const size_t dg = g->col_rows[slot_var[real[a0]]].size();
+      while (a1 < real.size() && g->col_rows[slot_var[real[a1]]].size() == dg) ++a1;
+      const int c = (int)(a1 - a0);
+      auto delta = [&](int q, int s) {
+        const auto &ra = g->col_rows[slot_var[real[a0 + q]]], &rb = g->col_rows[slot_var[real[a0 + q + s]]];
+        const int d0 = rb[0] - ra[0];
+        for (size_t t = 1; t < dg; ++t)
+          if (rb[t] - ra[t] != d0) return 0;
+        return d0 > 0 ? d0 : 0;
+      };
+      int along = 0;
+      for (int q = 0; q + 1 < c; ++q) along += delta(q, 1) == 1;
+      for (int s = 2; s <= 256 && 2 * s <= c && 2 * along < c - 1; ++s) {
+        if (c % s) continue;
+        const int d0 = delta(0, s);
+        bool all = d0 > 0 && ((m % d0 == 0 && (m / d0) % 32 == 0) || (d0 % 32 == 0 && m % 32 == 0)) && (sc == 0 || sc == d0);
+        for (int q = 1; q + s < c && all; ++q) all = delta(q, s) == d0;
+        if (!all) continue;
+        sc = d0;
+        for (int r0 = 0; r0 < s; ++r0)
+          for (int q = 0; q < c / s; ++q) sv2[real[a0 + (size_t)r0 * (c / s) + q]] = slot_var[real[a0 + (size_t)q * s + r0]];
+        break;
+      }
+      a0 = a1;
+    }
+    if (sc) {
+      const long long c_id = fill(+1);
+      fill(-1);
+      std::vector<int> lab2(m);
+      const int X = m / sc;
+      for (int i = 0; i < m; ++i)
+        lab2[i] = sc % 32 == 0 ? (i & ~31) + ((i & 31) + (i >> 5)) % 32
+                               : (i % sc) * X + (i / sc + i % sc) % X;
+      std::swap(lab, lab2);
+      std::swap(slot_var, sv2);
+      const long long c_tr = fill(+1);
+      fill(-1);
+      if (c_tr >= c_id) {
+        std::swap(lab, lab2);
+        std::swap(slot_var, sv2);
+      }
+      for (int p : real) posof[slot_var[p]] = p;
+    }
+  }
+  fill(+1);
+  std::vector<int> chk_of(m);
+  for (int i = 0; i < m; ++i) chk_of[lab[i]] = i;
+  uint64_t rs = 0x9E3779B97F4A7C15ull;
+  auto rnd = [&]() { rs ^= rs << 13; rs ^= rs >> 7; rs ^= rs << 17; return rs; };
+  auto take = [&](long long d, long long) { return d <= 0; };
+  for (long long it = 0; it < iters; ++it) {
+    if ((rnd() & 3u) != 0 && it % rot_every != 0) {
+      if (real.size() < 2) continue;
+      const int pa = real[rnd() % real.size()], pb = real[rnd() % real.size()];
+      const int ja = slot_var[pa], jb = slot_var[pb];
+      if (pa / 16 == pb / 16 || g->col_rows[ja].size() != g->col_rows[jb].size()) continue;
+      long long d = var_at(ja, pa, -1) + var_at(jb, pb, -1);
+      d += var_at(jb, pa, +1) + var_at(ja, pb, +1);
+      if (take(d, it)) {
+        slot_var[pa] = jb;
+        slot_var[pb] = ja;
+        posof[ja] = pb;
+        posof[jb] = pa;
+      } else {
+        var_at(jb, pa, -1), var_at(ja, pb, -1);
+        var_at(ja, pa, +1), var_at(jb, pb, +1);
+      }
+    } else if (it % rot_every == 0) {
+      const int q0 = (int)(rnd() % (uint64_t)((m + 31) / 32)) * 32, nb = std::min(32, m - q0);
+      const int sft = 1 + (int)(rnd() % (uint64_t)(nb > 1 ? nb - 1 : 1));
+      if (nb < 2) continue;
+      int blk[32];
+      for (int i = 0; i < nb; ++i) blk[i] = chk_of[q0 + i];
+      long long d = 0;
+      for (int i = 0; i < nb; ++i) d += check_as(blk[i], q0 + i, -1);
+      for (int i = 0; i < nb; ++i) d += check_as(blk[i], q0 + (i + sft) % nb, +1);
+      if (take(d, it)) {
+        for (int i = 0; i < nb; ++i) {
+          lab[blk[i]] = q0 + (i + sft) % nb;
+          chk_of[q0 + (i + sft) % nb] = blk[i];
+        }
+      } else {
+        for (int i = 0; i < nb; ++i) check_as(blk[i], q0 + (i + sft) % nb, -1);
+        for (int i = 0; i < nb; ++i) check_as(blk[i], q0 + i, +1);
+      }
+    } else {
+      const int a = (int)(rnd() % (uint64_t)m), b = (int)(rnd() % (uint64_t)m);
+      const int la = lab[a], lb = lab[b];
+      if ((la & 31) == (lb & 31)) continue;
+      long long d = check_as(a, la, -1) + check_as(b, lb, -1);
+      d += check_as(a, lb, +1) + check_as(b, la, +1);
+      if (take(d, it)) {
+        lab[a] = lb;
+        lab[b] = la;
+        chk_of[lb] = a;
+        chk_of[la] = b;
+      } else {
+        check_as(a, lb, -1), check_as(b, la, -1);
+        check_as(a, la, +1), check_as(b, lb, +1);
+      }
+    }
+  }
+  std::lock_guard<std::mutex> lk(memo_mu);
+  if (memo.size() >= kMemo) memo.clear();
+  memo[key] = {lab, slot_var};
+}
+
+static void pm_edges(const qldpc_graph* g, const Route& r, const std::vector<int32_t>& slot_var, const std::vector<int>& lab,
+                     std::vector<uint32_t>& out) {
+  const int TB = r.TB, VPL = r.VPL, DM = r.DMAX, stride = 256 * r.pm;
+  out.assign((size_t)VPL * DM * TB, kNoEdgeS);
+  for (int k = 0; k < VPL; ++k)
+    for (int t = 0; t < TB; ++t) {
+      const int j = slot_var[(size_t)k * TB + t];
+      if (j < 0) continue;
+      const auto& rows = g->col_rows[j];
+      for (int d = 0; d < (int)rows.size(); ++d) {
+        const int i = rows[d], l = lab.empty() ? i : lab[i];
+        const int32_t* b = g->col_idx.data() + g->row_ptr[i];
+        const int pos = (int)(std::lower_bound(b, g->col_idx.data() + g->row_ptr[i + 1], (int32_t)j) - b);
+        out[((size_t)k * DM + d) * TB + t] = (uint32_t)(l + 1) | ((uint32_t)(2 + pos * stride + l) << 16);
+      }
+    }
+}
+
 static int build_tables(qldpc_bp* bp, HostTables& T) {
   const qldpc_graph* g = bp->g;
   const Route& r = bp->route;
@@ -1336,11 +1557,16 @@
     T.lab = label_checks(g, r, bp->slot_var, &bp->gather_conf[0], &bp->gather_conf[1]);
   const bool f64e3 = r.engine == 3 && r.precision == 64 && r.m2s != 3;
   int ndummy = 0;
-  build_slot_edges(g, r, bp->slot_var, T.edges, (r.engine == 3 && env_int("QLDPC_BANKOPT", 1) != 0) ? (int)(L.v / 4) : -1,
-                   T.lab, r.m2s == 1 && env_int("QLDPC_M2S_PLACE", 1) != 0,
-                   r.vslots_dummy ? (1 + g->m * r.nch) * (16 / tsize) : -1, &ndummy,
-                   !f64e3 ? 0 : (r.m2s || r.tail) ? 1 : env_int("QLDPC_ANNEAL_2W", 1) != 0 ? 2 : 0, -1,
-                   (r.tail && r.vslots_dummy) ? (int)(L.t - L.v) / tsize : -1);
+  if (r.pm) {
+    pm_place(g, r, bp->slot_var, T.lab, -1);
+    pm_edges(g, r, bp->slot_var, T.lab, T.edges);
+  } else {
+    build_slot_edges(g, r, bp->slot_var, T.edges, (r.engine == 3 && env_int("QLDPC_BANKOPT", 1) != 0) ? (int)(L.v / 4) : -1,
+                     T.lab, r.m2s == 1 && env_int("QLDPC_M2S_PLACE", 1) != 0,
+                     r.vslots_dummy ? (1 + g->m * r.nch) * (16 / tsize) : -1, &ndummy,
+                     !f64e3 ? 0 : (r.m2s || r.tail) ? 1 : env_int("QLDPC_ANNEAL_2W", 1) != 0 ? 2 : 0, -1,
+                     (r.tail && r.vslots_dummy) ? (int)(L.t - L.v) / tsize : -1);
+  }
   if (ndummy != r.vslots_dummy) return set_err(QLDPC_EINVAL, "m2s private dummy slot count mismatch");
   if (f64e3 && r.ea_shift == 0) lds_model_var_phase(T.edges, r, L.v, bp->lds_model);
   if (r.m2s == 3)
@@ -1584,6 +1810,27 @@
   return 0;
 }
 
+int qldpc_m2s_pm_place(const qldpc_graph* g, int32_t anneal_iters, int32_t* geom4, int32_t* lab, int32_t* slot_var,
+                       int32_t slot_cap, uint32_t* edges, int32_t edge_cap, int64_t* out6) {
+  if (!g || !geom4 || !lab || !slot_var || !edges || !out6) return set_err(QLDPC_EINVAL, "NULL argument");
+  Route r;
+  std::vector<int32_t> sv;
+  if (const int rc = plan_route(g, true, 64, 0, 0, 0, r, sv)) return rc;
+  if (!r.pm) return set_err(QLDPC_ENOTSUP, "graph outside the position-major m2s envelope (QLDPC_M2S_PM, rows <= 7, m <= 768)");
+  if ((int)sv.size() > slot_cap || r.VPL * r.DMAX * r.TB > edge_cap) return set_err(QLDPC_EINVAL, "output arrays too small");
+  std::vector<int> lb;
+  pm_place(g, r, sv, lb, anneal_iters);
+  std::vector<uint32_t> ed;
+  pm_edges(g, r, sv, lb, ed);
+  lds_model_var_phase(ed, r, route_layout(r, route_vslots(r, g->m), g->m).v, out6);
+  const int32_t gm[4] = {r.TB, r.VPL, r.d3k, r.pm};
+  std::copy(gm, gm + 4, geom4);
+  for (int i = 0; i < g->m; ++i) lab[i] = lb.empty() ? i : lb[i];
+  std::copy(sv.begin(), sv.end(), slot_var);
+  std::copy(ed.begin(), ed.end(), edges);
+  return 0;
+}
+
 int qldpc_bp_bank_stats(const qldpc_bp* bp, int32_t* before, int32_t* after) {
   if (!bp) return set_err(QLDPC_EINVAL, "NULL decoder");
   if (before) *before = bp->gather_conf[0];
@@ -1789,7 +2036,7 @@
                       (dec_z && dec_z->route.tail && (!dec_z->route.m2s || dec_z->route.nch == 4)) ||
                       (dec_x && dec_z &&
                        (dec_x->route.m2s != dec_z->route.m2s || dec_x->route.tail != dec_z->route.tail || dec_x->route.fb != dec_z->route.fb ||
-                        dec_x->route.m2s_pk != dec_z->route.m2s_pk)) ||
+                        dec_x->route.m2s_pk != dec_z->route.m2s_pk || dec_x->route.pm != dec_z->route.pm)) ||
                       (dec_x && dec_z && dec_x->route.m2s && dec_x->route.d3k != dec_z->route.d3k) ||
                       env_int("QLDPC_MC_STAGED", 0) == 1;
   if (staged) return mc_create_staged(dec_x, logical_x, dec_z, logical_z, out);
@@ -1997,15 +2244,15 @@
     if (nchunks > 0x7fffffffLL) return set_err(QLDPC_EINVAL, "too many shots for one launch (chunk count >= 2^31)");
     const long long grid = std::max<long long>(1, std::min<long long>(nchunks, want));
     a.cls_cache = nullptr;
-    const size_t cc_need = (size_t)grid * (size_t)a.chunk * (size_t)mc->route.TB * 2;
-    if (a.nsec == 2 && !d_uniforms && mc->route.VPL <= 8 && env_int("QLDPC_CLS_CACHE", 1) != 0 && cc_need <= (256u << 20)) {
+    const size_t cc_need = (size_t)grid * (size_t)a.chunk * (size_t)a.sec[0].n;
+    if (a.nsec == 2 && !d_uniforms && env_int("QLDPC_CLS_CACHE", 1) != 0 && cc_need <= (256u << 20)) {
       const size_t need = cc_need;
       if (mc->cls_cache.bytes < need) {
         mc->cls_cache.release();
         int rc = mc->cls_cache.alloc(need);
         if (rc) return rc;
       }
-      a.cls_cache = static_cast<uint16_t*>(mc->cls_cache.p);
+      a.cls_cache = static_cast<uint8_t*>(mc->cls_cache.p);
     }
     hipStream_t st = (hipStream_t)stream;
     if (bposd) {
diff --git a/qldpc_fault_tolerance_amd/csrc/route.h b/qldpc_fault_tolerance_amd/csrc/route.h
--- a/qldpc_fault_tolerance_amd/csrc/route.h
+++ b/qldpc_fault_tolerance_amd/csrc/route.h
@@ -15,6 +15,7 @@
   int ea_shift = 0;
   int tail = 0;
   int m2s = 0;
+  int pm = 0;
   int fb = 0;
   int m2s_pk = 0;
   int vslots_dummy = 0;
@@ -26,6 +27,7 @@
 };
 
 inline int route_vslots(const Route& r, int m) {
+  if (r.pm) return 2 + 7 * 256 * r.pm;
   return r.vslots_m2v ? r.vslots_m2v : (1 + m * r.nch) * (r.precision == 32 ? 4 : 2) + r.vslots_dummy;
 }
 
diff --git a/qldpc_fault_tolerance_amd/csrc/variants.h b/qldpc_fault_tolerance_amd/csrc/variants.h
--- a/qldpc_fault_tolerance_amd/csrc/variants.h
+++ b/qldpc_fault_tolerance_amd/csrc/variants.h
@@ -49,6 +49,9 @@
 SVariant get_rvariant_f32_st(int vpl, int d3k);
 SVariant get_rvariant_f64_m2st(int vpl, int d3k, int d2k);
 SVariant get_rvariant_f64_m2s(int vpl, int d3k);
+SVariant get_rvariant_f64_m2sp1(int vpl, int d3k);
+SVariant get_rvariant_f64_m2sp2(int vpl, int d3k);
+SVariant get_rvariant_f64_m2sp3(int vpl, int d3k);
 SVariant get_rvariant_f64_m2s8(int vpl, int d3k);
 SVariant get_rvariant_f64_m2s8pk(int vpl, int d3k);
 SVariant get_rvariant_f64_m2v(int vpl, int d3k);
```

After: 1.281 million (median of 6 runs). Within noise of the previous version (+0.4%).
